# facebookresearch/SlowFast

Measured on AMD Instinct MI355X. Metric: clips/sec (fwd+bwd), SlowFast-8x8-R50 32x224^2 synthetic clips, per-GPU batch 32, higher is better.
Workload: dtype fp16; 1 GPU; SLOWFAST_8x8_R50: forward + cross_entropy loss + backward + sgd step, inputs resident in HBM, per-GPU batch 32; global_batch=32, parallelism=dp1, launch=hip-graph(fwd+bwd) + eager all-reduce/optimizer, optimizer=FlatOptimizer (fused unscale+norm+clip+update, dynamic loss scale on device)

## Files before the change

### include/sfamd.h

```cpp
#ifndef SFAMD_H
#define SFAMD_H
#include <stddef.h>
#include <stdint.h>
#ifdef __cplusplus
extern "C" {
#endif

#define SF_ABI_VERSION 34
typedef void* sf_stream_t;

typedef struct sf_conv_desc {
    int32_t N, Ci, Ti, Hi, Wi;
    int32_t Co, To, Ho, Wo;
    int32_t kT, kH, kW;
    int32_t sT, sH, sW;
    int32_t pT, pH, pW;
    int32_t dT, dH, dW;
    int32_t Cw;
    int32_t ldx, ldy;
    int32_t Cow;
} sf_conv_desc;

int sf_abi_version(void);
const char* sf_backend(void);
#define SF_ACT_FP16 0
#define SF_ACT_BF16_ID 1
int sf_act_dtype(void);
const char* sf_last_error(void);
const char* sf_build_id(void);

int sf_conv_weight_ld(const sf_conv_desc* d, int32_t* ldf, int32_t* ldd);
int sf_prep_weights(const sf_conv_desc* d, const float* w, void* wf, void* wd, sf_stream_t stream);
typedef struct sf_prep_item {
    const float* w;
    void* wf;
    void* wd;
    int32_t Co, Cow, Cw, Cp, taps, ldf, ldd;
    int32_t pad;
} sf_prep_item;
int sf_prep_item_fill(const sf_conv_desc* d, const float* w, void* wf, void* wd, sf_prep_item* item);
int64_t sf_prep_item_blocks(const sf_prep_item* item);
int sf_prep_weights_batch(const sf_prep_item* items, const int32_t* blk_item, const int32_t* blk_off, int32_t nblocks,
                          sf_stream_t stream);
int sf_conv_fwd_mtiles(const sf_conv_desc* d);
int sf_conv_fwd(const sf_conv_desc* d, const void* x, const void* wf, const float* in_scale, const float* in_shift,
                int in_relu, const float* bias, void* y, float* stat_part, sf_stream_t stream);
int sf_conv_fwd_fused(const sf_conv_desc* d, const void* x, const void* wf, const float* bias, const void* resid,
                      int32_t ldr, int out_relu, void* y, sf_stream_t stream);
int sf_conv_dgrad(const sf_conv_desc* d, const void* dy, const void* wd, const void* resid, int32_t ldr,
                  const void* resid_bits, void* dx, sf_stream_t stream);
int sf_conv_dgrad_bn(const sf_conv_desc* d, const void* dy, const void* wd, const void* resid, int32_t ldr,
                     const void* resid_bits, void* dx, const float* mask_scale, const float* mask_shift,
                     const void* mask_bits, const void* bn_y, int32_t bn_ldy, float* bn_part, int32_t bn_part_rows,
                     int32_t* bn_rows, sf_stream_t stream);
int64_t sf_conv_wgrad_workspace(const sf_conv_desc* d);
int64_t sf_conv_wgrad_rowtab_bytes(const sf_conv_desc* d);
int sf_conv_wgrad_rowtab(const sf_conv_desc* d, void* tab, sf_stream_t stream);
int sf_conv_wgrad(const sf_conv_desc* d, const void* x, const float* in_scale, const float* in_shift, int in_relu,
                  const void* dy, float* dw, float out_scale, int zero_first, void* workspace, int64_t workspace_bytes,
                  const void* rowtab, sf_stream_t stream);
int sf_conv_c_bwd_plan(const sf_conv_desc* d, int in_affine, int mask_bits, int32_t* tile_rows, int64_t* workspace_bytes);
int sf_conv_c_bwd(const sf_conv_desc* d, const void* dz, int32_t lddz, const void* mask_bits, const void* yc, int32_t ldyc,
                  const float* coef, const void* act, const void* wd, const float* bn_scale, const float* bn_shift,
                  const void* bn_y, int32_t bn_ldy, float* bn_part, int32_t bn_part_rows, int32_t* bn_rows, void* d_in,
                  int32_t ld_in, float* dw, float out_scale, int zero_first, void* workspace, int64_t workspace_bytes,
                  sf_stream_t stream);

int sf_bn_finalize(float* part, int32_t nblk, int32_t C, int32_t Creal, float count, const float* gamma, const float* beta,
                   float* running_mean, float* running_var, float momentum, float eps, float* scale, float* shift,
                   float* save_mean, float* save_rstd, sf_stream_t stream);
int sf_bn_act(int64_t M, int32_t C, const void* y, int32_t ldy, const float* scale, const float* shift, const void* r,
              int32_t ldr, const float* rscale, const float* rshift, int relu, void* out, int32_t ldo, void* mask_out,
              sf_stream_t stream);
int sf_bn_bwd_blocks(int64_t M, int32_t C);
int sf_bn_bwd_reduce(int64_t M, int32_t C, const void* dz, int32_t lddz, const void* zmask, int32_t ldm, const void* y,
                     int32_t ldy, const float* scale, const float* shift, int relu_self, float* part,
                     sf_stream_t stream);
int sf_bn_bwd_finalize(float* part, int32_t nblk, int32_t C, int32_t Creal, float count, const float* gamma, const float* mean,
                       const float* rstd, float inv_loss_scale, float* dgamma, float* dbeta, int accumulate,
                       float* coef, sf_stream_t stream);
int sf_bn_bwd_apply(int64_t M, int32_t C, const void* dz, int32_t lddz, const void* zmask, int32_t ldm, const void* y,
                    int32_t ldy, const float* scale, const float* shift, int relu_self, const float* coef, void* dy,
                    int32_t lddy, void* gout, int32_t ldg, sf_stream_t stream);

int sf_pool_fwd(int32_t N, int32_t T, int32_t H, int32_t W, int32_t C, int32_t kH, int32_t kW, int32_t sH, int32_t sW,
                int32_t pH, int32_t pW, const void* y, int32_t ldy, const float* scale, const float* shift, int relu,
                void* out, int32_t ldo, void* argmax, int32_t cls, sf_stream_t stream);
int sf_pool_bwd(int32_t N, int32_t T, int32_t H, int32_t W, int32_t C, int32_t kH, int32_t kW, int32_t sH, int32_t sW,
                int32_t pH, int32_t pW, const void* pooled, int32_t ldp, const void* argmax, int relu,
                const void* dout, int32_t lddo, void* g, int32_t ldg, int32_t cls, sf_stream_t stream);

int sf_pool3d_fwd(int32_t N, int32_t T, int32_t H, int32_t W, int32_t C, int32_t kT, int32_t kH, int32_t kW, const void* x,
                  int32_t ldx, void* out, int32_t ldo, void* argmax, sf_stream_t stream);
int sf_pool3d_bwd(int32_t N, int32_t T, int32_t H, int32_t W, int32_t C, int32_t kT, int32_t kH, int32_t kW,
                  const void* argmax, const void* dout, int32_t lddo, void* dx, int32_t lddx, sf_stream_t stream);

int sf_ncthw_to_cl(const float* x, int32_t N, int32_t C, int64_t S, int32_t Cp, void* out, sf_stream_t stream);
int sf_cl_to_ncthw(const void* x, int32_t ld, int32_t N, int32_t C, int64_t S, float* out, sf_stream_t stream);


int sf_bgemm(int64_t M, int32_t N, int32_t K, const void* A, int32_t lda, const void* W, int32_t ldw, const float* bias,
             const void* resid, int32_t ldr, void* Y, int32_t ldy, int32_t nbatch, int32_t bh, int64_t sa_b, int64_t sa_h,
             int64_t sw_b, int64_t sw_h, int64_t sy_b, int64_t sy_h, int64_t sr_b, int64_t sr_h, int32_t resid_row0,
             float alpha, sf_stream_t stream);
typedef struct sf_rows32 {
    const float* in;
    float* out;
    int32_t ld, period;
} sf_rows32;
int sf_gemm_rows32(int64_t M, int32_t N, int32_t K, const void* A, int32_t lda, const void* W, int32_t ldw, const float* bias,
                   const void* resid, int32_t ldr, void* Y, int32_t ldy, const sf_rows32* side, sf_stream_t stream);
int sf_bgemm_tn(int64_t M, int32_t R, int32_t Kc, const void* P, int32_t ldp, const void* X, int32_t ldx, void* Out,
                int32_t ldo, float scale, int32_t nbatch, int32_t bh, int64_t sp_b, int64_t sp_h, int64_t sx_b,
                int64_t sx_h, int64_t so_b, int64_t so_h, sf_stream_t stream);

int sf_layernorm_fwd(int64_t M, int32_t C, const void* x, int32_t ldx, const float* gamma, const float* beta, float eps,
                     void* y, int32_t ldy, float* mean, float* rstd, sf_stream_t stream);
int sf_layernorm_fwd_rows32(int64_t M, int32_t C, const void* x, int32_t ldx, const float* gamma, const float* beta, float eps,
                            void* y, int32_t ldy, float* mean, float* rstd, const sf_rows32* side, sf_stream_t stream);
int sf_layernorm_bwd_blocks(int64_t M, int32_t C);
int sf_layernorm_bwd(int64_t M, int32_t C, const void* dy, int32_t lddy, const void* x, int32_t ldx, const float* gamma,
                     const float* mean, const float* rstd, const void* resid, int32_t ldr, void* dx, int32_t lddx,
                     float* part, sf_stream_t stream);
int sf_layernorm_bwd_sums(int64_t M, int32_t C, const void* dy, int32_t lddy, const void* x, int32_t ldx, const float* gamma,
                          const float* mean, const float* rstd, const void* resid, int32_t ldr, void* dx, int32_t lddx,
                          float* part, sf_stream_t stream);
int sf_colsum_blocks(int64_t M, int32_t C);
int sf_colsum(int64_t M, int32_t C, const void* x, int32_t ldx, float* part, sf_stream_t stream);
int sf_colsum_finalize(float* part, int32_t nblk, int32_t C, int32_t fold, float* out0, float* out1, float scale,
                       int accumulate, sf_stream_t stream);
typedef struct sf_colfin_item {
    float* part;
    int32_t nblk, C, fold;
    float* out0;
    float* out1;
    float scale;
    int32_t accumulate;
    int32_t row_stride;
} sf_colfin_item;
int sf_colsum_finalize_batch(const sf_colfin_item* items, int32_t n, sf_stream_t stream);
int sf_rows_sum(const float* part, int32_t nblk, int64_t row_len, int64_t offset, int32_t n, float* out, float scale,
                int accumulate, sf_stream_t stream);
int sf_gelu_fwd(int64_t n, const void* h, void* a, sf_stream_t stream);
int sf_gelu_bwd(int64_t n, const void* h, const void* da, void* dh, sf_stream_t stream);

typedef struct sf_dw_desc {
    int32_t N, C, Cw, cls;
    int32_t Ti, Hi, Wi, To, Ho, Wo;
    int32_t kT, kH, kW, sT, sH, sW, pT, pH, pW;
// ... 196 lines not shown
```

### slowfast_amd/csrc/sf_api.hip

```cpp
#include "../../include/sfamd.h"
#include "sf_bn.h"
#include "sf_common.h"
#include "sf_igemm.h"
#include "sf_igemm2.h"
#include "sf_wgrad2.h"
#include "sf_cbwd.h"
#include "sf_pool.h"
#include "sf_dwconv.h"
#include "sf_dwsweep.h"
#include "sf_dwtemporal.h"
#include "sf_tokens.h"
#include "sf_x3d.h"
#include "sf_stem.h"
#include "sf_attn.h"
#include "sf_roi.h"
#include "sf_optim.h"
#include "sf_mixup.h"
#include "sf_erase.h"
#include "sf_pack.h"
#include "sf_sample.h"
#include "sf_color.h"
#include "sf_randaug.h"
#include "sf_sslcolor.h"
#include "sf_hog.h"
// ... 541 lines not shown
        }
    }
    IgemmParams p = gemm_params(gather_fwd(d, x, nullptr, nullptr, 0), d->N * d->To * d->Ho * d->Wo, wf, ldf, d->Co,
                                y, d->ldy, bias, resid, ldr);
    p.act_mode = out_relu ? 3 : 0;
    return run_igemm(p, is_pointwise(d), (hipStream_t)stream);
}

struct BnFuse {
    const float* scale; const float* shift; const void* bits;
    const void* y0; int32_t ld0; float* part0;
};
static int conv_dgrad_impl(const sf_conv_desc* d, const void* dy, const void* wd, const void* resid, int32_t ldr,
                           const void* resid_bits, void* dx, const BnFuse* bn, int32_t* bn_rows, sf_stream_t stream) {
    if (check_desc(d)) return -1;
    REQUIRE(dy && wd && dx, "sf_conv_dgrad: null pointer");
    REQUIRE(!resid || (ldr >= d->Ci && ldr % 8 == 0), "sf_conv_dgrad: bad residual pitch");
    int32_t ldf, ldd;
    sf_conv_weight_ld(d, &ldf, &ldd);
    IgemmParams p = gemm_params(gather_dgrad(d, dy), d->N * d->Ti * d->Hi * d->Wi, wd, ldd, d->Ci, dx, d->ldx, nullptr, resid, ldr);
    REQUIRE(!resid_bits || resid, "sf_conv_dgrad: resid_bits without a residual");
    p.resid_bits = (const uint8_t*)resid_bits;
    const bool fuse = bn && d->sT == 1 && d->sH == 1 && d->sW == 1;
    if (!resid && d->Co == 8 && d->To == d->Ti && d->Ho == d->Hi && d->Wo == d->Wi) {
        sf_conv_desc dd = *d;
        dd.Ci = d->Co; dd.Cw = d->Co; dd.Co = d->Ci; dd.Cow = 0;
        dd.pT = d->kT - 1 - d->pT; dd.pH = d->kH - 1 - d->pH; dd.pW = d->kW - 1 - d->pW;
        dd.ldx = d->ldy; dd.ldy = d->ldx;
        const StemPlan sp = plan_stem_fwd(&dd, true, fuse, cdiv(p.M, 128), fuse);
        if (sp.ok) {
            StemParams q = stem_fwd_params(&dd, sp, dy, wd, ldd, dx);
            const int S = d->kT * d->kH;
            q.wo0 = ((S - 1) * 3 + 2) * 8; q.wos = -24; q.wog = -8; q.kwc = 3;
            if (fuse) {
                q.bnb_y = (const f16*)bn->y0; q.bnb_ld = bn->ld0; q.bnb_scale = bn->scale; q.bnb_shift = bn->shift;
                q.bnb_bits = (const uint8_t*)bn->bits;
                q.stat_part = bn->part0; q.stat_rows = 0;
            }
            launch_stem_fwd(sp, q, (hipStream_t)stream);
            if (bn_rows) *bn_rows = fuse ? sp.ntiles : 0;
            return check_launch("stem_dgrad");
        }
    }
    if (fuse) {
        p.bnb_y = (const f16*)bn->y0; p.bnb_ld = bn->ld0; p.bnb_part = bn->part0;
        p.bnb_scale = bn->scale; p.bnb_shift = bn->shift; p.bnb_bits = (const uint8_t*)bn->bits;
    }
    GemmPlan g;
    const int rc = run_igemm(p, is_pointwise(d), (hipStream_t)stream, &g);
    if (bn_rows) *bn_rows = (fuse && g.bm > 0) ? cdiv(p.M, g.bm) : 0;
    return rc;
}

extern "C" int sf_conv_dgrad(const sf_conv_desc* d, const void* dy, const void* wd, const void* resid, int32_t ldr,
                             const void* resid_bits, void* dx, sf_stream_t stream) {
    return conv_dgrad_impl(d, dy, wd, resid, ldr, resid_bits, dx, nullptr, nullptr, stream);
}

extern "C" int sf_conv_dgrad_bn(const sf_conv_desc* d, const void* dy, const void* wd, const void* resid, int32_t ldr,
                                const void* resid_bits, void* dx, const float* mask_scale, const float* mask_shift,
                                const void* mask_bits, const void* bn_y, int32_t bn_ldy, float* bn_part, int32_t bn_part_rows,
                                int32_t* bn_rows, sf_stream_t stream) {
    REQUIRE(d && bn_y && bn_part && bn_rows, "sf_conv_dgrad_bn: null pointer");
    REQUIRE(mask_bits || (mask_scale && mask_shift), "sf_conv_dgrad_bn: a mask source is needed (mask_bits, or mask_scale + mask_shift)");
    REQUIRE(bn_ldy >= d->Ci && bn_ldy % 8 == 0 && ((uintptr_t)bn_y & 15) == 0, "sf_conv_dgrad_bn: bad bn_y pitch / alignment");
    REQUIRE((int64_t)bn_part_rows * 128 >= (int64_t)d->N * d->Ti * d->Hi * d->Wi,
            "sf_conv_dgrad_bn: the partial table needs ceil(positions / 128) rows of [2][Ci] floats");
    const BnFuse bn = {mask_scale, mask_shift, mask_bits, bn_y, bn_ldy, bn_part};
    return conv_dgrad_impl(d, dy, wd, resid, ldr, resid_bits, dx, &bn, bn_rows, stream);
}

static inline int wgrad1_bmw(int rows) { return rows >= 128 ? 128 : rows >= 64 ? 64 : rows >= 32 ? 32 : 16; }
static inline int wgrad1_ks(int bmw) { return bmw <= 32 ? 4 : 1; }
static void launch_wgrad1(int bmw, WgradParams& p, dim3 grid3, hipStream_t s) {
    p.tiles_k = grid3.x; p.tiles_c = grid3.y;
    const dim3 grid(grid3.x * grid3.y * grid3.z), block(SF_THREADS);
    switch (bmw) {
        case 128: hipLaunchKernelGGL((sf_wgrad_kernel<128, 64, 64, 1>), grid, block, 0, s, p); break;
        case 64: hipLaunchKernelGGL((sf_wgrad_kernel<64, 32, 64, 1>), grid, block, 0, s, p); break;
        case 32: hipLaunchKernelGGL((sf_wgrad_kernel<32, 32, 32, 4>), grid, block, 0, s, p); break;
        default: hipLaunchKernelGGL((sf_wgrad_kernel<16, 16, 32, 4>), grid, block, 0, s, p); break;
    }
}
static void launch_wgrad_reduce(const sf_conv_desc* d, const float* ws, int slabs, int Co_pad, int Kpad, bool slice4, float* dw,
                                float out_scale, int zero_first, hipStream_t s) {
    WgradReduceParams r;
    memset(&r, 0, sizeof(r));
    r.ws = ws; r.splits = slabs; r.Co = d->Cow ? d->Cow : d->Co; r.Co_pad = Co_pad; r.Kpad = Kpad;
    r.taps = d->kT * d->kH * d->kW; r.Ktot = r.taps * d->Ci; r.fdC = make_fastdiv(d->Ci); r.dw = dw; r.Cw = d->Cw;
    if (slice4) { r.slice4 = 1; r.Ktot = d->kT * d->kH * 32; }
    r.out_scale = out_scale; r.accumulate = zero_first ? 0 : 1;
    const int64_t total = (int64_t)r.Co * r.Kpad / 4;
    r.lanes = 1;
    while (r.lanes < 32 && r.lanes * 4 <= r.splits) r.lanes *= 2;
    hipLaunchKernelGGL(sf_wgrad_reduce_kernel, dim3(cdiv(total, SF_THREADS / r.lanes)), dim3(SF_THREADS), 0, s, r);
}

enum WgradPath { WGRAD_GEN1, WGRAD_ROWTAB, WGRAD_STEM };
struct WgradPlan {
    WgradPath path;
    bool thin, dual;
    int BMW, BKW, KS, tiles_k, tiles_c, Co_pad, Kpad;
    int nchunks, chunks_per_split;
    int rows_per_split, splits;
    int slabs;
    size_t tab_bytes, ws_bytes;
    StemPlan stem;
};
static WgradPlan plan_wgrad1(const sf_conv_desc* d) {
    WgradPlan w;
    memset(&w, 0, sizeof(w));
    w.path = WGRAD_GEN1;
    const int taps = d->kT * d->kH * d->kW;
    const int Ktot = taps * d->Ci;
    const int64_t M = (int64_t)d->N * d->To * d->Ho * d->Wo;
    w.BMW = wgrad1_bmw(d->Co); w.KS = wgrad1_ks(w.BMW);
    w.tiles_k = cdiv(Ktot, 128);
    w.tiles_c = cdiv(d->Co, w.BMW);
    w.Kpad = w.tiles_k * 128;
    w.Co_pad = w.tiles_c * w.BMW;
    w.nchunks = cdiv(M, 32);
    const int64_t slab = (int64_t)w.Co_pad * w.Kpad * 4;
    static const int target = tune_knob("SF_WGRAD_BLOCKS", 1024);
    int splits = cdiv(target, (int64_t)w.tiles_k * w.tiles_c);
    const int64_t cap = (256ll << 20) / slab;
    if (splits > cap) splits = (int)(cap < 1 ? 1 : cap);
    const int nstages = cdiv(w.nchunks, w.KS);
    if (splits > nstages) splits = nstages;
    if (splits < 1) splits = 1;
    w.chunks_per_split = cdiv(nstages, splits) * w.KS;
    w.splits = cdiv(w.nchunks, w.chunks_per_split);
    w.slabs = w.splits;
    w.ws_bytes = (size_t)slab * w.splits;
    return w;
}

static bool plan_wgrad2(const sf_conv_desc* d, WgradPlan& w) {
    if (test_hook("SF_WGRAD2", 1) == 0) return false;
    const int mink = test_hook("SF_WGRAD2_MINK", 192);
    const int minrows = test_hook("SF_WGRAD2_MINROWS", 4096);
    const int taps = d->kT * d->kH * d->kW;
    const int target = test_hook("SF_WGRAD2_BLOCKS", 512);
    const int Ktot = taps * d->Ci;
    const int64_t M = (int64_t)d->N * d->To * d->Ho * d->Wo;
    if (taps > SF_I2_MAXTAPS || M < minrows) return false;
    if ((d->kT - 1) * d->dT > 127 || (d->kH - 1) * d->dH > 127 || (d->kW - 1) * d->dW > 127) return false;
    if (d->Co <= 32) {
        if (test_hook("SF_WGRAD2T", 1) == 0) return false;
        const int minrows_t = test_hook("SF_WGRAD2T_MINROWS", 16384);
        if (M < minrows_t) return false;
        w.thin = true;
        w.BMW = d->Co <= 16 ? 16 : 32;
        w.BKW = Ktot <= 32 ? 32 : 128;
        w.tiles_k = cdiv(Ktot, w.BKW);
        w.tiles_c = 1;
        w.Kpad = w.tiles_k * w.BKW;
        w.Co_pad = w.BMW;
        const int target_t = test_hook("SF_WGRAD2T_BLOCKS", w.BKW == 128 ? 512 : w.BMW == 32 ? 768 : 1024);
        int splits = target_t / w.tiles_k;
        if (splits < 1) splits = 1;
        w.rows_per_split = roundup(cdiv(M, splits), 128);
        w.splits = cdiv(M, w.rows_per_split);
        w.tab_bytes = ((size_t)M * 8 + 255) / 256 * 256 + 1280;
        w.ws_bytes = w.tab_bytes + (size_t)w.Co_pad * w.Kpad * 4 * w.splits;
        w.slabs = w.splits;
        w.path = WGRAD_ROWTAB;
        return true;
    }
    if (Ktot < mink) return false;
    w.BMW = d->Co > 64 ? 128 : 64;
    w.tiles_k = cdiv(Ktot, 256);
    w.tiles_c = cdiv(d->Co, w.BMW);
    w.Kpad = w.tiles_k * 256;
    w.Co_pad = w.tiles_c * w.BMW;
    int splits = target / (w.tiles_k * w.tiles_c);
    const int64_t slab = (int64_t)w.Co_pad * w.Kpad * 4;
    const int64_t cap = (256ll << 20) / slab;
    if (splits > cap) splits = (int)(cap < 1 ? 1 : cap);
    if (splits < 1) splits = 1;
    w.dual = false;
    if (splits >= 2 && test_hook("SF_WGRAD2_DUAL", 1) != 0) {
        const int tiles = w.tiles_k * w.tiles_c;
        const int pairs = (target / 2) / tiles;
        const int64_t steps = cdiv(cdiv(M, splits), 32);
        if (pairs >= 1 && 2 * pairs * 10 >= (2 * pairs < splits ? splits : 2 * pairs) * 9 && steps <= test_hook("SF_WGRAD2_DUAL_STEPS", 80)) {
            w.dual = true;
            if (2 * pairs < splits) splits = 2 * pairs;
        }
    }
    w.rows_per_split = roundup(cdiv(M, splits), 32);
    w.splits = cdiv(M, w.rows_per_split);
    if (w.splits < 2) w.dual = false;
    w.slabs = w.dual ? cdiv(w.splits, 2) : w.splits;
    w.tab_bytes = ((size_t)M * 8 + 255) / 256 * 256 + 1280;
    w.ws_bytes = w.tab_bytes + (size_t)slab * w.splits;
    w.path = WGRAD_ROWTAB;
    return true;
}
static WgradPlan plan_conv_wgrad(const sf_conv_desc* d, bool in_affine) {
    const StemPlan sp = plan_stem(d);
    WgradPlan w;
    memset(&w, 0, sizeof(w));
    if (in_affine || !(sp.ok || plan_wgrad2(d, w))) w = plan_wgrad1(d);
    else if (sp.ok) {
        w.path = WGRAD_STEM;
        w.slabs = sp.wg_blocks * sp.wgroups; w.Co_pad = 16; w.Kpad = sp.Kpad; w.ws_bytes = sp.ws_bytes;
    }
    w.stem = sp;
    return w;
}

static void launch_rowtab(const sf_conv_desc* d, void* tab, hipStream_t s) {
    RowtabParams t;
    memset(&t, 0, sizeof(t));
    t.tab = (i32x2*)tab;
    t.M = d->N * d->To * d->Ho * d->Wo;
    t.fdW = make_fastdiv(d->Wo); t.fdH = make_fastdiv(d->Ho); t.fdT = make_fastdiv(d->To);
    t.sT = d->Ti; t.sH = d->Hi; t.sW = d->Wi;
    t.strT = d->sT; t.strH = d->sH; t.strW = d->sW; t.padT = d->pT; t.padH = d->pH; t.padW = d->pW;
    t.ntaps = d->kT * d->kH * d->kW;
    int ti = 0;
    for (int kt = 0; kt < d->kT; ++kt)
        for (int kh = 0; kh < d->kH; ++kh)
            for (int kw = 0; kw < d->kW; ++kw, ++ti) {
                t.dt[ti] = (int8_t)(kt * d->dT); t.dh[ti] = (int8_t)(kh * d->dH); t.dw[ti] = (int8_t)(kw * d->dW);
            }
    hipLaunchKernelGGL(sf_wgrad2_rowtab_kernel, dim3(cdiv(t.M, SF_THREADS)), dim3(SF_THREADS), 0, s, t);
}

extern "C" int64_t sf_conv_wgrad_rowtab_bytes(const sf_conv_desc* d) {
    if (check_desc(d)) return -1;
    return (int64_t)plan_conv_wgrad(d, false).tab_bytes;
}

extern "C" int sf_conv_wgrad_rowtab(const sf_conv_desc* d, void* tab, sf_stream_t stream) {
    if (check_desc(d)) return -1;
    REQUIRE(tab && (uintptr_t)tab % 16 == 0, "sf_conv_wgrad_rowtab: tab must be a 16-byte aligned device pointer");
    REQUIRE(plan_conv_wgrad(d, false).path == WGRAD_ROWTAB, "sf_conv_wgrad_rowtab: this geometry does not take the row-table kernel (sf_conv_wgrad_rowtab_bytes == 0)");
    launch_rowtab(d, tab, (hipStream_t)stream);
    return check_launch("wgrad_rowtab");
}

extern "C" int64_t sf_conv_wgrad_workspace(const sf_conv_desc* d) {
    if (check_desc(d)) return -1;
    const int64_t plain = (int64_t)plan_conv_wgrad(d, false).ws_bytes, affine = (int64_t)plan_conv_wgrad(d, true).ws_bytes;
    return plain > affine ? plain : affine;
}

extern "C" int sf_conv_wgrad(const sf_conv_desc* d, const void* x, const float* in_scale, const float* in_shift,
                             int in_relu, const void* dy, float* dw, float out_scale, int zero_first,
                             void* workspace, int64_t workspace_bytes, const void* rowtab, sf_stream_t stream) {
    if (check_desc(d)) return -1;
    REQUIRE(x && dy && dw && workspace, "sf_conv_wgrad: null pointer");
    REQUIRE((in_scale == nullptr) == (in_shift == nullptr), "sf_conv_wgrad: in_scale/in_shift must come together");
    REQUIRE(!in_scale || d->Ci <= 512, "sf_conv_wgrad: fused input BatchNorm supports Ci <= 512 (got %d)", d->Ci);
    hipStream_t s = (hipStream_t)stream;
    GatherSide gk = gather_fwd(d, x, in_scale, in_shift, in_relu);
    const WgradPlan w = plan_conv_wgrad(d, in_scale != nullptr);
    REQUIRE(workspace_bytes >= (int64_t)w.ws_bytes, "sf_conv_wgrad: workspace too small (%lld < %lld bytes)",
            (long long)workspace_bytes, (long long)w.ws_bytes);
    float* slabs = (float*)((char*)workspace + w.tab_bytes);
    if (w.path == WGRAD_ROWTAB) {
        REQUIRE(((uintptr_t)x | (uintptr_t)dy | (uintptr_t)workspace) % 16 == 0, "sf_conv_wgrad: operands must be 16-byte aligned");
        Wgrad2Params q;
        memset(&q, 0, sizeof(q));
        int ti = 0;
        for (int kt = 0; kt < d->kT; ++kt)
            for (int kh = 0; kh < d->kH; ++kh)
                for (int kw = 0; kw < d->kW; ++kw, ++ti) q.dlin[ti] = (kt * d->dT * d->Hi + kh * d->dH) * d->Wi + kw * d->dW;
        if (!rowtab) launch_rowtab(d, workspace, s);
        else REQUIRE((uintptr_t)rowtab % 16 == 0, "sf_conv_wgrad: rowtab must be 16-byte aligned");
        q.x = (const f16*)x; q.ldx = d->ldx; q.C = d->Ci;
        q.dy = (const f16*)dy; q.ldy = d->ldy; q.Co = d->Co;
        q.M = d->N * d->To * d->Ho * d->Wo; q.Ktot = gk.Ktot;
        q.rowtab = (const i32x2*)(rowtab ? rowtab : workspace);
        q.ws = slabs; q.Co_pad = w.Co_pad; q.Kpad = w.Kpad;
        q.tiles_k = w.tiles_k; q.tiles_c = w.tiles_c; q.rows_per_split = w.rows_per_split;
        q.stage_stride = (w.thin && tune_knob("SF_WGRAD2T_RR", 1) != 0) ? w.splits : 0;
        const dim3 grid((unsigned)(w.tiles_k * w.tiles_c * w.slabs));
        if (sf_trace()) fprintf(stderr, "[sfamd] wgrad2: M=%d Co=%d K=%d tiles %dx%d splits %d%s\n", q.M, q.Co, q.Ktot, w.tiles_c, w.tiles_k, w.splits,
                                w.dual ? " (two per workgroup)" : "");
        if (w.thin) {
            if (w.BMW == 16 && w.BKW == 128) hipLaunchKernelGGL((sf_wgrad2t_kernel<16, 128, 2>), grid, dim3(256), 0, s, q);
            else if (w.BMW == 32 && w.BKW == 128) hipLaunchKernelGGL((sf_wgrad2t_kernel<32, 128, 2>), grid, dim3(256), 0, s, q);
            else if (w.BMW == 16) hipLaunchKernelGGL((sf_wgrad2t_kernel<16, 32, 3>), grid, dim3(256), 0, s, q);
            else hipLaunchKernelGGL((sf_wgrad2t_kernel<32, 32, 3>), grid, dim3(256), 0, s, q);
        } else if (w.dual) {
            if (w.BMW == 128) hipLaunchKernelGGL((sf_wgrad2_kernel<128, true>), grid, dim3(1024), 0, s, q);
            else hipLaunchKernelGGL((sf_wgrad2_kernel<64, true>), grid, dim3(1024), 0, s, q);
        } else {
            if (w.BMW == 128) hipLaunchKernelGGL((sf_wgrad2_kernel<128>), grid, dim3(512), 0, s, q);
            else hipLaunchKernelGGL((sf_wgrad2_kernel<64>), grid, dim3(512), 0, s, q);
        }
    } else if (w.path == WGRAD_STEM) {
        const StemPlan& sp = w.stem;
        StemParams q = stem_params(d, sp, x);
        q.dy = (const f16*)dy; q.ws = (float*)workspace;
        if (sf_trace()) fprintf(stderr, "[sfamd] stem_wgrad: %d workgroups x %d tiles\n", sp.wg_blocks, sp.tiles_per_block);
        static const bool stem_plain = tune_knob("SF_STEM_XCD", 1) == 0;
        q.plain_order = stem_plain ? 1 : 0;
        const dim3 grid(sp.wg_blocks), block(SF_STEM_WG_THREADS);
        if (d->Co <= 8 && sp.small) hipLaunchKernelGGL((sf_stem_wgrad_kernel<8, SF_STEM_CHUNKS_SMALL>), grid, block, 0, s, q);
        else if (d->Co <= 8) hipLaunchKernelGGL((sf_stem_wgrad_kernel<8, SF_STEM_CHUNKS>), grid, block, 0, s, q);
        else if (sp.small) hipLaunchKernelGGL((sf_stem_wgrad_kernel<16, SF_STEM_CHUNKS_SMALL>), grid, block, 0, s, q);
        else hipLaunchKernelGGL((sf_stem_wgrad_kernel<16, SF_STEM_CHUNKS>), grid, block, 0, s, q);
    } else {
        REQUIRE(w.splits <= 65535, "sf_conv_wgrad: too many splits");
        WgradParams p;
        memset(&p, 0, sizeof(p));
        p.g = gk;
        p.dy = (const f16*)dy; p.ldy = d->ldy; p.Co = d->Co;
        p.M = d->N * d->To * d->Ho * d->Wo;
        p.ws = (float*)workspace; p.Co_pad = w.Co_pad; p.Kpad = w.Kpad;
        p.nchunks = w.nchunks; p.chunks_per_split = w.chunks_per_split;
        launch_wgrad1(w.BMW, p, dim3(w.tiles_k, w.tiles_c, w.splits), s);
    }
    if (check_launch("wgrad")) return -1;
    launch_wgrad_reduce(d, slabs, w.slabs, w.Co_pad, w.Kpad, w.path == WGRAD_STEM && w.stem.thin3, dw, out_scale, zero_first, s);
    return check_launch("wgrad_reduce");
}

struct CbwdPlan {
    bool ok;
    int cip, cop, R;
    size_t ws_bytes;
};
#define SF_CBWD_MAX_WGS 1024
template <int CIP, int COP>
static void cbwd_fill(CbwdPlan& w) {
    using K = CbwdCfg<CIP, COP>;
    w.R = K::R;
    w.ws_bytes = (size_t)SF_CBWD_MAX_WGS * COP * CIP * 4;
}
#define SF_CBWD_FOR_SHAPE(cip, cop, ...)                                                         \
    do {                                                                                         \
        if ((cip) == 16 && (cop) == 32) { constexpr int CIP_ = 16, COP_ = 32; __VA_ARGS__; }            \
        else if ((cip) == 16 && (cop) == 64) { constexpr int CIP_ = 16, COP_ = 64; __VA_ARGS__; }       \
        else if ((cip) == 16 && (cop) == 128) { constexpr int CIP_ = 16, COP_ = 128; __VA_ARGS__; }     \
        else if ((cip) == 16 && (cop) == 256) { constexpr int CIP_ = 16, COP_ = 256; __VA_ARGS__; }     \
        else if ((cip) == 32 && (cop) == 32) { constexpr int CIP_ = 32, COP_ = 32; __VA_ARGS__; }       \
        else if ((cip) == 32 && (cop) == 64) { constexpr int CIP_ = 32, COP_ = 64; __VA_ARGS__; }       \
        else if ((cip) == 32 && (cop) == 128) { constexpr int CIP_ = 32, COP_ = 128; __VA_ARGS__; }     \
        else if ((cip) == 32 && (cop) == 256) { constexpr int CIP_ = 32, COP_ = 256; __VA_ARGS__; }     \
        else if ((cip) == 64 && (cop) == 32) { constexpr int CIP_ = 64, COP_ = 32; __VA_ARGS__; }       \
        else if ((cip) == 64 && (cop) == 64) { constexpr int CIP_ = 64, COP_ = 64; __VA_ARGS__; }       \
        else if ((cip) == 64 && (cop) == 128) { constexpr int CIP_ = 64, COP_ = 128; __VA_ARGS__; }     \
        else { constexpr int CIP_ = 64, COP_ = 256; __VA_ARGS__; }                                      \
    } while (0)
static CbwdPlan plan_cbwd(const sf_conv_desc* d, bool in_affine, bool mask_bits) {
    CbwdPlan w;
    memset(&w, 0, sizeof(w));
    if (test_hook("SF_CBWD", 1) == 0) return w;
    if (d->kT != 1 || d->kH != 1 || d->kW != 1 || d->sT != 1 || d->sH != 1 || d->sW != 1 || d->pT || d->pH || d->pW) return w;
    if (d->To != d->Ti || d->Ho != d->Hi || d->Wo != d->Wi) return w;
    if (d->Ci % 8 || d->Ci > 64 || d->Co % 32 || d->Co > 256) return w;
    if (in_affine || !mask_bits) return w;
    w.cip = d->Ci <= 16 ? 16 : d->Ci <= 32 ? 32 : 64;
    w.cop = d->Co <= 32 ? 32 : d->Co <= 64 ? 64 : d->Co <= 128 ? 128 : 256;
    SF_CBWD_FOR_SHAPE(w.cip, w.cop, (cbwd_fill<CIP_, COP_>(w)));
    w.ok = true;
    return w;
}

extern "C" int sf_conv_c_bwd_plan(const sf_conv_desc* d, int in_affine, int mask_bits, int32_t* tile_rows,
                                  int64_t* workspace_bytes) {
    if (check_desc(d)) return -1;
    const CbwdPlan w = plan_cbwd(d, in_affine != 0, mask_bits != 0);
    if (tile_rows) *tile_rows = w.ok ? 128 : 0;
    if (workspace_bytes) *workspace_bytes = w.ok ? (int64_t)w.ws_bytes : 0;
    return w.ok ? 1 : 0;
}

extern "C" int sf_conv_c_bwd(const sf_conv_desc* d, const void* dz, int32_t lddz, const void* mask_bits, const void* yc,
                             int32_t ldyc, const float* coef, const void* act, const void* wd, const float* bn_scale,
                             const float* bn_shift, const void* bn_y, int32_t bn_ldy, float* bn_part, int32_t bn_part_rows,
                             int32_t* bn_rows, void* d_in, int32_t ld_in, float* dw, float out_scale, int zero_first,
                             void* workspace, int64_t workspace_bytes, sf_stream_t stream) {
    if (check_desc(d)) return -1;
    REQUIRE(dz && mask_bits && yc && coef && act && wd && d_in && dw && workspace, "sf_conv_c_bwd: null pointer");
    const CbwdPlan w = plan_cbwd(d, false, true);
    REQUIRE(w.ok, "sf_conv_c_bwd: this geometry keeps sf_bn_bwd_apply + sf_conv_wgrad + sf_conv_dgrad_bn (sf_conv_c_bwd_plan == 0)");
    REQUIRE(lddz >= d->Co && lddz % 8 == 0 && ldyc >= d->Co && ldyc % 8 == 0 && ld_in >= d->Ci && ld_in % 8 == 0,
            "sf_conv_c_bwd: bad row pitch");
    REQUIRE((((uintptr_t)dz | (uintptr_t)yc | (uintptr_t)act | (uintptr_t)wd | (uintptr_t)d_in | (uintptr_t)workspace) & 15) == 0,
            "sf_conv_c_bwd: operands must be 16-byte aligned");
    REQUIRE(workspace_bytes >= (int64_t)w.ws_bytes, "sf_conv_c_bwd: workspace too small (%lld < %lld bytes)",
            (long long)workspace_bytes, (long long)w.ws_bytes);
    const int64_t M = (int64_t)d->N * d->Ti * d->Hi * d->Wi;
    const int ntiles = cdiv(M, 128);
    const bool fuse = bn_part != nullptr;
    if (fuse) {
        REQUIRE(bn_scale && bn_shift && bn_y && bn_rows, "sf_conv_c_bwd: the fused reduction needs bn_scale, bn_shift, bn_y and bn_rows");
        REQUIRE(bn_ldy >= d->Ci && bn_ldy % 8 == 0 && ((uintptr_t)bn_y & 15) == 0, "sf_conv_c_bwd: bad bn_y pitch / alignment");
        REQUIRE(bn_part_rows >= ntiles, "sf_conv_c_bwd: the partial table needs ceil(positions / tile_rows) rows of [2][Ci] floats");
    }
    int32_t ldf, ldd;
    sf_conv_weight_ld(d, &ldf, &ldd);
    CbwdParams p;
    memset(&p, 0, sizeof(p));
    p.M = (int)M; p.Ci = d->Ci; p.Co = d->Co;
    p.dz = (const f16*)dz; p.lddz = lddz; p.bits = (const uint8_t*)mask_bits; p.yc = (const f16*)yc; p.ldyc = ldyc;
    p.coef = coef; p.act = (const f16*)act; p.ldact = d->ldx; p.wd = (const f16*)wd; p.ldw = ldd;
    if (fuse) { p.bnb_y = (const f16*)bn_y; p.bnb_ld = bn_ldy; p.bnb_scale = bn_scale; p.bnb_shift = bn_shift; p.bnb_part = bn_part; }
    p.dx = (f16*)d_in; p.lddx = ld_in; p.ws = (float*)workspace; p.tiles128 = ntiles;
    int wgs;
    const WgradPlan w2 = plan_conv_wgrad(d, false);
    const int forced = test_hook("SF_CBWD_WGS", 0);
    if (forced > 0) {
        wgs = forced < SF_CBWD_MAX_WGS ? forced : SF_CBWD_MAX_WGS;
        p.rps = roundup(cdiv(M, wgs), 32);
        wgs = cdiv(M, p.rps);
    } else if (w2.path == WGRAD_ROWTAB && w2.thin && w2.splits <= SF_CBWD_MAX_WGS) {
        wgs = w2.splits; p.rps = 0;
    } else {
        const WgradPlan w1 = plan_wgrad1(d);
        wgs = w1.splits; p.rps = w1.chunks_per_split * 32;
        REQUIRE(wgs <= SF_CBWD_MAX_WGS, "sf_conv_c_bwd: %d splits", wgs);
    }
    hipStream_t s = (hipStream_t)stream;
    SF_CBWD_FOR_SHAPE(w.cip, w.cop, hipLaunchKernelGGL((sf_cbwd_kernel<CIP_, COP_>), dim3(wgs), dim3(SF_THREADS), 0, s, p));
    if (check_launch("conv_c_bwd")) return -1;
    if (bn_rows) *bn_rows = fuse ? ntiles : 0;
    launch_wgrad_reduce(d, (const float*)workspace, wgs, w.cop, w.cip, false, dw, out_scale, zero_first, s);
    return check_launch("conv_c_bwd_reduce");
}

static RowTile make_rowtile(int64_t M, int C, int max_blocks, dim3& grid) {
    RowTile rt;
    rt.M = (int)M; rt.C = C;
    const int G = C / 8;
    const int TG = G < SF_THREADS ? G : SF_THREADS;
    const int rpi = SF_THREADS / TG;
    int passes = cdiv(M, (int64_t)rpi * max_blocks);
    if (passes < 1) passes = 1;
    rt.rows_per_block = rpi * passes;
    grid = dim3(cdiv(M, rt.rows_per_block), cdiv(G, SF_THREADS));
    return rt;
}
static int check_rows(const char* who, int64_t M, int C) {
    REQUIRE(M > 0 && M < (1ll << 31), "%s: bad row count", who);
    REQUIRE(C > 0 && C % 8 == 0, "%s: C must be a positive multiple of 8 (got %d)", who, C);
    return 0;
}

static const int kFoldAbove = tune_knob("SF_FOLD_ABOVE", 2048);
static int fold_partials(float* part, int& nblk, int C, hipStream_t s) {
    if (nblk <= kFoldAbove || nblk <= 256) return 1;
    const int group = nblk <= 2048 ? 16 : nblk <= 8192 ? 32 : 64;
    const int cols = 2 * C;
    dim3 grid(cdiv(cols, SF_THREADS), cdiv(nblk, group));
    hipLaunchKernelGGL(sf_part_fold_kernel, grid, dim3(SF_THREADS), 0, s, part, nblk, cols, group);
    nblk = cdiv(nblk, group);
    return group;
}

extern "C" int sf_bn_finalize(float* part, int32_t nblk, int32_t C, int32_t Creal, float count, const float* gamma,
                              const float* beta, float* running_mean, float* running_var, float momentum, float eps,
                              float* scale, float* shift, float* save_mean, float* save_rstd, sf_stream_t stream) {
    REQUIRE(gamma && beta && scale && shift, "sf_bn_finalize: null pointer");
    REQUIRE(nblk > 0 ? part != nullptr : (running_mean && running_var), "sf_bn_finalize: missing statistics source");
    REQUIRE(Creal > 0 && Creal <= C, "sf_bn_finalize: Creal must be in (0, C]");
    BnFinalizeParams p;
    p.row_stride = nblk > 0 ? fold_partials(part, nblk, C, (hipStream_t)stream) : 1;
    p.part = part; p.nblk = nblk; p.C = C; p.Creal = Creal; p.count = count; p.gamma = gamma; p.beta = beta;
    p.running_mean = running_mean; p.running_var = running_var; p.momentum = momentum; p.eps = eps;
    p.scale = scale; p.shift = shift; p.save_mean = save_mean; p.save_rstd = save_rstd;
    hipLaunchKernelGGL(sf_bn_finalize_kernel, dim3(cdiv(C, SF_FIN_CH)), dim3(sf_fin_threads(p.nblk)), 0, (hipStream_t)stream, p);
    return check_launch("bn_finalize");
}

extern "C" int sf_bn_act(int64_t M, int32_t C, const void* y, int32_t ldy, const float* scale, const float* shift,
                         const void* r, int32_t ldr, const float* rscale, const float* rshift, int relu, void* out,
                         int32_t ldo, void* mask_out, sf_stream_t stream) {
    if (check_rows("sf_bn_act", M, C)) return -1;
    REQUIRE(y && out, "sf_bn_act: null pointer");
    BnActParams p;
    dim3 grid;
    p.rt = make_rowtile(M, C, 8192, grid);
    p.y = (const f16*)y; p.ldy = ldy; p.scale = scale; p.shift = shift;
    p.r = (const f16*)r; p.ldr = ldr; p.rscale = rscale; p.rshift = rshift;
    p.relu = relu; p.out = (f16*)out; p.ldo = ldo; p.mask_out = (uint8_t*)mask_out;
    hipLaunchKernelGGL(sf_bn_act_kernel, grid, dim3(SF_THREADS), 0, (hipStream_t)stream, p);
    return check_launch("bn_act");
}

static const int kBwdBlocks = tune_knob("SF_BN_BWD_BLOCKS", 1024);
extern "C" int sf_bn_bwd_blocks(int64_t M, int32_t C) {
    if (check_rows("sf_bn_bwd_blocks", M, C)) return -1;
    dim3 grid;
    make_rowtile(M, C, kBwdBlocks, grid);
    return (int)grid.x;
}

extern "C" int sf_bn_bwd_reduce(int64_t M, int32_t C, const void* dz, int32_t lddz, const void* zmask, int32_t ldm,
                                const void* y, int32_t ldy, const float* scale, const float* shift, int relu_self,
                                float* part, sf_stream_t stream) {
    if (check_rows("sf_bn_bwd_reduce", M, C)) return -1;
    REQUIRE(dz && y && part, "sf_bn_bwd_reduce: null pointer");
    REQUIRE(!relu_self || (scale && shift), "sf_bn_bwd_reduce: relu_self needs scale/shift");
    BnBwdReduceParams p;
    dim3 grid;
    p.rt = make_rowtile(M, C, kBwdBlocks, grid);
    p.dz = (const f16*)dz; p.lddz = lddz; p.zmask = (const f16*)zmask; p.ldm = ldm;
    p.y = (const f16*)y; p.ldy = ldy; p.scale = scale; p.shift = shift; p.relu_self = relu_self; p.part = part;
    hipLaunchKernelGGL(sf_bn_bwd_reduce_kernel, grid, dim3(SF_THREADS), 0, (hipStream_t)stream, p);
    return check_launch("bn_bwd_reduce");
}
// ... 2379 lines not shown
```

### slowfast_amd/csrc/sf_igemm.h

```cpp
#pragma once
#include "sf_common.h"

struct IgemmParams {
    GatherSide g;
    int M;
    const f16* wmat;
    int ldw;
    int Nout;
    int ksteps;
    f16* y;
    int ldy;
    const float* bias;
    const f16* resid;
    int ldr;
    float* stat_part;
    int ntiles_n;
    int bh;
    int64_t sa_b, sa_h, sw_b, sw_h, sy_b, sy_h, sr_b, sr_h;
    int act_mode;
    f16* act_aux;
    int ld_aux;
    int resid_row0;
    const uint8_t* resid_bits;
    float alpha;
// ... 320 lines not shown
            ok[u] = idx < BM * CG && m < p.M && ecol < p.Nout;
            rok[u] = ok[u] && resid && m >= p.resid_row0;
            if constexpr (F32R) {
                uint32_t srow;
                if (f32_row(p.f32, m, srow)) rok[u] = false;
            }
            L[u].rbits = 0xffu; L[u].bbits = 0u;
            if (rok[u]) {
                L[u].r = ld16(resid + (int64_t)m * p.ldr + ecol);
                if (p.resid_bits) L[u].rbits = p.resid_bits[(int64_t)m * (p.Nout >> 3) + (ecol >> 3)];
            }
            if (ok[u] && bnb && p.bnb_y) {
                L[u].y = ld16(p.bnb_y + (int64_t)m * p.bnb_ld + ecol);
                if (p.bnb_bits) L[u].bbits = p.bnb_bits[(int64_t)m * (p.Nout >> 3) + (ecol >> 3)];
            }
        }
#pragma unroll
        for (int u = 0; u < CH; ++u) {
            if (!ok[u]) continue;
            const int idx = tid + (it0 + u) * SF_THREADS;
            const int row = idx / CG, m = m0 + row;
            f16x8 v = ld16(stg + row * STG_LD + ecg * 8);
            if (rok[u]) {
#pragma unroll
                for (int e = 0; e < 8; ++e) {
                    const f16 r = ((L[u].rbits >> e) & 1u) ? L[u].r[e] : (f16)0.f;
                    v[e] = (f16)((float)v[e] + (float)r);
                }
            }
            if (p.act_mode == 2) {
                const f16x8 h = ld16(p.act_aux + (int64_t)m * p.ld_aux + ecol);
#pragma unroll
                for (int e = 0; e < 8; ++e) v[e] = (f16)((float)v[e] * gelu_df((float)h[e]));
            }
            if (p.act_mode == 3) {
#pragma unroll
                for (int e = 0; e < 8; ++e) v[e] = v[e] > (f16)0.f ? v[e] : (f16)0.f;
            }
            st16(yout + (int64_t)m * p.ldy + ecol, v);
            if (p.act_mode == 1) {
                f16x8 a;
#pragma unroll
                for (int e = 0; e < 8; ++e) a[e] = (f16)gelu_f((float)v[e]);
                st16(p.act_aux + (int64_t)m * p.ld_aux + ecol, a);
            }
            if (bnb && p.bnb_y) bnb_accumulate(v, L[u].y, bsc, bsh, bsg, bsgy, p.bnb_bits != nullptr, L[u].bbits);
            else if (bnb) {
#pragma unroll
                for (int e = 0; e < 8; ++e) bsg[e] += (float)v[e];
            }
        }
    }
    if (bnb) bnb_reduce_store<4, CG>(bsg, bsgy, reinterpret_cast<float*>(smem), p.bnb_part + (int64_t)mt * 2 * p.Nout, n0, p.Nout);
}

struct WgradParams {
    GatherSide g;
    const f16* dy;
    int ldy;
    int Co;
    int M;
    float* ws;
    int Co_pad, Kpad;
    int nchunks;
    int chunks_per_split;
    int tiles_k, tiles_c;
    int bh;
    int64_t sp_b, sp_h, sx_b, sx_h, so_b, so_h;
    f16* out16; int ldo; float out_scale;
};

struct WgradReduceParams {
    const float* ws;
    int splits, Co, Co_pad, Kpad, Ktot;
    FastDiv fdC;
    float* dw;
    int Cw, taps;
    float out_scale;
    int accumulate;
    int lanes;
    int slice4;
};

__global__ __launch_bounds__(SF_THREADS) void sf_wgrad_reduce_kernel(WgradReduceParams p) {
    __shared__ f32x4 s_acc[SF_THREADS];
    const int L = p.lanes, E = SF_THREADS / L;
    const int e = threadIdx.x % E, z0 = threadIdx.x / E;
    const int64_t total = (int64_t)p.Co * p.Kpad;
    const int64_t slab = (int64_t)p.Co_pad * p.Kpad;
    const int64_t idx = ((int64_t)blockIdx.x * E + e) * 4;
    f32x4 a0 = {0.f, 0.f, 0.f, 0.f}, a1 = a0, a2 = a0, a3 = a0;
    if (idx < total) {
        const float* src = p.ws + idx;
        int z = z0;
        for (; z + 3 * L < p.splits; z += 4 * L) {
            const f32x4 v0 = *reinterpret_cast<const f32x4*>(src + (int64_t)z * slab);
            const f32x4 v1 = *reinterpret_cast<const f32x4*>(src + (int64_t)(z + L) * slab);
            const f32x4 v2 = *reinterpret_cast<const f32x4*>(src + (int64_t)(z + 2 * L) * slab);
            const f32x4 v3 = *reinterpret_cast<const f32x4*>(src + (int64_t)(z + 3 * L) * slab);
            a0 += v0; a1 += v1; a2 += v2; a3 += v3;
        }
        for (; z < p.splits; z += L) a0 += *reinterpret_cast<const f32x4*>(src + (int64_t)z * slab);
    }
    s_acc[threadIdx.x] = (a0 + a1) + (a2 + a3);
    __syncthreads();
    for (int half = L >> 1; half >= 1; half >>= 1) {
        if (z0 < half) s_acc[threadIdx.x] += s_acc[threadIdx.x + half * E];
        __syncthreads();
    }
    if (z0 == 0 && idx < total) {
        const int co = (int)(idx / p.Kpad), kcol0 = (int)(idx % p.Kpad);
        const f32x4 r = s_acc[threadIdx.x];
#pragma unroll
        for (int j = 0; j < 4; ++j) {
            const int kcol = kcol0 + j;
            if (kcol < p.Ktot) {
                uint32_t tap, ci;
                fd_divmod((uint32_t)kcol, p.fdC, tap, ci);
                if (p.slice4) {
                    if ((tap & 3u) == 3u) continue;
                    tap = (tap >> 2) * 3u + (tap & 3u);
                }
                if (ci < (uint32_t)p.Cw) {
                    float* dst = p.dw + ((int64_t)co * p.Cw + ci) * p.taps + tap;
                    const float v = r[j] * p.out_scale;
                    *dst = p.accumulate ? *dst + v : v;
                }
            }
        }
    }
}

template <class V>
__device__ __forceinline__ f16x4 as_f16x4(V v) {
    f16x4 o;
    __builtin_memcpy(&o, &v, 8);
    return o;
}

struct TapPos {
    int dt, dh, dw;
    uint32_t c0;
    bool valid;
};
__device__ __forceinline__ TapPos decode_tap(const GatherSide& g, uint32_t k0) {
    TapPos t;
    t.valid = k0 < (uint32_t)g.Ktot;
    uint32_t tap, kt, kh, kw, q;
    fd_divmod(t.valid ? k0 : 0u, g.fdC, tap, t.c0);
    fd_divmod(tap, g.fdkW, q, kw);
    fd_divmod(q, g.fdkH, kt, kh);
    t.dt = (int)kt * g.dilT; t.dh = (int)kh * g.dilH; t.dw = (int)kw * g.dilW;
    return t;
}
__device__ __forceinline__ bool gather_offset_tap(const GatherSide& g, const RowPos& r, const TapPos& tp, int64_t& off) {
    if (!r.valid || !tp.valid) return false;
    const int t = r.bt + tp.dt, h = r.bh + tp.dh, w = r.bw + tp.dw;
    if ((unsigned)t >= (unsigned)g.sT || (unsigned)h >= (unsigned)g.sH || (unsigned)w >= (unsigned)g.sW) return false;
    off = ((((int64_t)r.n * g.sT + t) * g.sH + h) * g.sW + w) * (int64_t)g.ld + tp.c0;
    return true;
}

template <int BMW, int WM, int WN, int KS>
__global__ __launch_bounds__(SF_THREADS) void sf_wgrad_kernel(WgradParams p) {
    constexpr int BNW = 128, BKM = 32, ROWS = BKM * KS;
    constexpr int WAVES_N = BNW / WN, WAVES_M = BMW / WM;
    static_assert(WAVES_M * WAVES_N == 4, "4 waves per workgroup");
    constexpr int TM = WM / 16, TN = WN / 16;
    constexpr int LDA = BMW + 16, LDB = BNW + 16;
    constexpr int BUF = ROWS * (LDA + LDB);
    constexpr int NBUF = KS == 1 ? 2 : 1;
    constexpr int NA = (ROWS * (BMW / 8) + SF_THREADS - 1) / SF_THREADS;
    constexpr int NX = 2 * KS;

    __shared__ __attribute__((aligned(16))) f16 smem[NBUF * BUF];
    __shared__ __attribute__((aligned(16))) float s_scale[512];
    __shared__ __attribute__((aligned(16))) float s_shift[512];

    const int tid = threadIdx.x;
    const int lane = tid & 63, wave = tid >> 6;
    const int wm = wave / WAVES_N, wn = wave % WAVES_N;
    const uint32_t wg = xcd_remap(blockIdx.x, gridDim.x);
    const int bx = (int)(wg % (uint32_t)p.tiles_k);
    const int by = (int)((wg / (uint32_t)p.tiles_k) % (uint32_t)p.tiles_c);
    const int bz = (int)(wg / ((uint32_t)p.tiles_k * (uint32_t)p.tiles_c));
    const int n0 = bx * BNW, c0 = by * BMW;
    const GatherSide& g = p.g;
    const bool has_tf = g.scale != nullptr;
    if (has_tf) {
        for (int c = tid; c < g.C; c += SF_THREADS) {
            s_scale[c] = g.scale[c];
            s_shift[c] = g.shift[c];
        }
    }
    const f16* x_src = g.src;
    const f16* dy_src = p.dy;
    f16* out16 = p.out16;
    const int nstages = (p.nchunks + KS - 1) / KS;
    int sb = bz * (p.chunks_per_split / KS);
    int se = sb + p.chunks_per_split / KS;
    if (p.bh > 0) {
        const int zb = bz / p.bh, zj = bz % p.bh;
        dy_src += zb * p.sp_b + zj * p.sp_h;
        x_src += zb * p.sx_b + zj * p.sx_h;
        out16 += zb * p.so_b + zj * p.so_h;
        sb = 0;
        se = nstages;
    }
    if (se > nstages) se = nstages;

    f16x8 ra[NA], rb[NX];
    bool rb_ok[NX];
    const TapPos tp = decode_tap(g, (uint32_t)(n0 + (tid & 15) * 8));

// ... 125 lines not shown
```

### slowfast_amd/engine.py

```python
import functools
import os

import torch

from . import lib as _sflib

from . import ops

_f16 = _sflib.act_dtype()
_listeners = []
FORCE_WEIGHT_PREP = False
PARAM_EPOCH = 0
PACK_RECORD = None
PACK_PLAN = os.environ.get("SF_PACK_PLAN", "1") != "0"
BN_FUSE_REDUCE = os.environ.get("SF_BN_FUSE_REDUCE", "1") != "0"
CAT_IN_PLACE = os.environ.get("SF_CAT_IN_PLACE", "1") != "0"
SEGMENTS = None


class _Segments:
    def __init__(self):
        self.cuts = []

    def cut(self, tensors):
# ... 547 lines not shown
        N, Cs, T, H, W = x_s.shape
        Cf = yf.shape[1]
        assert tuple(yf.shape) == (N, Cf, T, H, W), "lateral connection does not match the Slow pathway shape"
        cat = getattr(x_s, "_sf_cat", None)
        if cat is not None and tuple(cat.shape) == (N, Cs + Cf, T, H, W) and cat.data_ptr() == x_s.data_ptr():
            pass
        else:
            cat = ops.cl_empty((N, Cs + Cf, T, H, W), x_s.device)
            ops.bn_act(x_s, out=cat[:, :Cs])
        ops.bn_act(yf, st.scale, st.shift, relu=True, out=cat[:, Cs:])
        if CAPTURE is not None:
            CAPTURE.append({"kind": "fuse", "mod": mod, "raw": [yf], "bn": [(st.scale, st.shift)]})
        ctx.mod, ctx.yf, ctx.st, ctx.Cs = mod, yf, st, Cs
        ctx.save_for_backward(x_f)
        return cat, x_f.view_as(x_f)

    @staticmethod
    @delivers_grads
    def backward(ctx, dcat, dxf):
        unit = ctx.mod._unit
        (x_f,) = ctx.saved_tensors
        dcat = as_cl(dcat)
        dyf = unit.bn_backward(dcat[:, ctx.Cs:], ctx.yf, ctx.st, relu_self=True)
        need_dx = ctx.needs_input_grad[1]
        dx_f = unit.backward(x_f, None, dyf, need_dx=need_dx, resid=as_cl(dxf) if dxf is not None else None)
        _notify(unit.params())
        ctx.yf = None
        dx_s = dcat[:, :ctx.Cs] if ctx.needs_input_grad[0] else None
        return (dx_s, dx_f, None) + param_grads(ctx, 3)


class ResBlockFn(torch.autograd.Function):

    @staticmethod
    def forward(ctx, x, mod, *params):
        record_params(ctx, params)
        ctx.prev_bn = getattr(x, "_sf_block_bn", None) if BN_FUSE_REDUCE else None
        x = as_cl(x)
        units, P = mod.branch2._chain, mod._proj
        tr = mod.training
        raw, bn, act, h = [], [], [], x
        for i, u in enumerate(units):
            h, st = u.forward(h, None, tr)
            raw.append(h)
            bn.append(st)
            if i + 1 < len(units):
                h = ops.bn_act(h, st.scale, st.shift, relu=True)
                act.append(h)
        yc, sc = raw[-1], bn[-1]
        out_view, cat = None, None
        extra = getattr(mod, "_cat_extra", 0)
        if extra and CAT_IN_PLACE:
            N_, C_, T_, H_, W_ = yc.shape
            cat = ops.cl_empty((N_, C_ + extra, T_, H_, W_), x.device)
            out_view = cat[:, :C_]
        if P is not None:
            y1, s1 = P.forward(x, None, tr)
            out, bits = ops.bn_act(yc, sc.scale, sc.shift, relu=True, resid=y1, rscale=s1.scale, rshift=s1.shift,
                                   want_mask=True, out=out_view)
        else:
            y1, s1 = None, None
            out, bits = ops.bn_act(yc, sc.scale, sc.shift, relu=True, resid=x, want_mask=True, out=out_view)
        if cat is not None:
            out._sf_cat = cat
        if CAPTURE is not None:
            CAPTURE.append({"kind": "resblock", "mod": mod, "raw": list(raw), "bn": [(b.scale, b.shift) for b in bn], "out": out})
        ctx.mod = mod
        ctx.raw = (raw, y1, act, bits)
        ctx.bn = (bn, s1)
        ctx.save_for_backward(x)
        if BN_FUSE_REDUCE and tr:
            out._sf_block_bn = {"bits": bits, "y0": yc, "sync": _sync_of(units[-1].bn) is not None}
        return out

    @staticmethod
    @delivers_grads
    def backward(ctx, dout):
        mod = ctx.mod
        units, P = mod.branch2._chain, mod._proj
        (x,) = ctx.saved_tensors
        raw, y1, act, bits = ctx.raw
        bn, s1 = ctx.bn
        last = len(units) - 1
        part_c = tagged_bn_part(dout, raw[last])
        dout = as_cl(dout)
        need_dx = ctx.needs_input_grad[0]
        cgeom = units[last].fused_c_geom(act[last - 1]) if last > 0 else None
        if cgeom is None:
            dy = units[last].bn_backward(dout, raw[last], bn[last], zmask=bits, part=part_c)
        if P is not None:
            dy1 = P.bn_backward(dout, y1, s1, zmask=bits)
        for i in range(last, 0, -1):
            part = None
            if i == last and cgeom is not None:
                inner = (raw[i - 1], bn[i - 1]) if BN_FUSE_REDUCE and _sync_of(units[i - 1].bn) is None else None
                d_in, part = units[i].fused_c_backward(cgeom, act[i - 1], dout, raw[i], bn[i], bits, part=part_c, bn_fuse=inner)
            elif BN_FUSE_REDUCE and _sync_of(units[i - 1].bn) is None:
                d_in, part = units[i].backward(act[i - 1], None, dy, need_dx=True, bn_fuse=(raw[i - 1], bn[i - 1]))
            else:
                d_in = units[i].backward(act[i - 1], None, dy, need_dx=True)
            dy = units[i - 1].bn_backward(d_in, raw[i - 1], bn[i - 1], relu_self=True, part=part)
        prev = ctx.prev_bn if need_dx else None
        if prev is not None and prev["sync"]:
            prev = None
        if P is not None:
            dx1 = P.backward(x, None, dy1, need_dx=need_dx)
            dx = units[0].backward(x, None, dy, need_dx=need_dx, resid=dx1, bn_fuse=prev)
        else:
            dx = units[0].backward(x, None, dy, need_dx=need_dx, resid=dout, resid_bits=bits, bn_fuse=prev)
        if prev is not None:
            dx, pc = dx
            if pc is not None:
                tag_bn_part(dx, prev["y0"], pc)
        _notify(mod._param_list)
        ctx.raw = ctx.bn = ctx.prev_bn = None
        return (dx, None) + param_grads(ctx, 2)


CUT_BACKWARD = False
_cut_bn_tags = {}


def retag_cut_grad(g):
    tag = _cut_bn_tags.pop(g.data_ptr(), None)
    if tag is not None and getattr(g, "_sf_bn_part", None) is None and tag[2] == g.data_ptr() and tag[3] == g._version:
        g._sf_bn_part = tag


def tag_bn_part(dx, y0, part):
    dx._sf_bn_part = (y0.data_ptr(), part, dx.data_ptr(), dx._version)
    if CUT_BACKWARD:
        _cut_bn_tags[dx.data_ptr()] = dx._sf_bn_part


def tagged_bn_part(dout, y0):
    tag = getattr(dout, "_sf_bn_part", None)
    if tag is None or tag[0] != y0.data_ptr() or tag[2] != dout.data_ptr() or tag[3] != dout._version:
        return None
    return tag[1]


class ConvBNActFn(torch.autograd.Function):

    @staticmethod
    def forward(ctx, x, unit, relu, training, *params):
        record_params(ctx, params)
        x = as_cl(x)
        y, st = unit.forward(x, None, training)
        out = ops.bn_act(y, st.scale, st.shift, relu=relu)
        if CAPTURE is not None:
            CAPTURE.append({"kind": "convbnact", "mod": None, "raw": [y], "bn": [(st.scale, st.shift)], "out": out})
        ctx.unit, ctx.relu, ctx.y, ctx.st = unit, relu, y, st
        ctx.save_for_backward(x)
        return out

    @staticmethod
    @delivers_grads
    def backward(ctx, dout):
        unit = ctx.unit
        (x,) = ctx.saved_tensors
        dy = unit.bn_backward(as_cl(dout), ctx.y, ctx.st, relu_self=ctx.relu)
        dx = unit.backward(x, None, dy, need_dx=ctx.needs_input_grad[0])
        _notify(unit.params())
        ctx.y = None
        return (dx, None, None, None) + param_grads(ctx, 4)
```

### slowfast_amd/lib.py

```python
import ctypes
import os
from ctypes import POINTER, Structure, c_char_p, c_float, c_int, c_int32, c_int64, c_void_p

_HERE = os.path.dirname(os.path.abspath(__file__))
ABI_VERSION = 34
ACT_MODE = os.environ.get("SF_ACT_DTYPE", "fp16").lower()
if ACT_MODE not in ("fp16", "bf16"):
    raise ValueError(f"SF_ACT_DTYPE={ACT_MODE!r}: expected fp16 or bf16")
DEFAULT_LIBRARY = os.path.join(_HERE, "libsfamd.so" if ACT_MODE == "fp16" else "libsfamd_bf16.so")


def act_dtype():
    import torch
    return torch.float16 if ACT_MODE == "fp16" else torch.bfloat16


def act_eps():
    return 2.0 ** -11 if ACT_MODE == "fp16" else 2.0 ** -8


class ConvDesc(Structure):

    _fields_ = [(n, c_int32) for n in (
        "N", "Ci", "Ti", "Hi", "Wi", "Co", "To", "Ho", "Wo", "kT", "kH", "kW", "sT", "sH", "sW",
        "pT", "pH", "pW", "dT", "dH", "dW", "Cw", "ldx", "ldy", "Cow")]


class PrepItem(Structure):

    _fields_ = [("w", c_void_p), ("wf", c_void_p), ("wd", c_void_p)] + [(n, c_int32) for n in (
        "Co", "Cow", "Cw", "Cp", "taps", "ldf", "ldd", "pad")]


class DwDesc(Structure):

    _fields_ = [(n, c_int32) for n in (
        "N", "C", "Cw", "cls", "Ti", "Hi", "Wi", "To", "Ho", "Wo", "kT", "kH", "kW", "sT", "sH", "sW",
        "pT", "pH", "pW", "ldx", "ldy", "Cwreal")]


class Rows32(Structure):

    _fields_ = [("in_", c_void_p), ("out", c_void_p), ("ld", c_int32), ("period", c_int32)]


class ColFinItem(Structure):

    _fields_ = [("part", c_void_p), ("nblk", c_int32), ("C", c_int32), ("fold", c_int32), ("out0", c_void_p),
                ("out1", c_void_p), ("scale", c_float), ("accumulate", c_int32), ("row_stride", c_int32)]


class AttnDesc(Structure):

    _fields_ = [(n, c_int32) for n in (
        "B", "heads", "D", "cls", "Nq", "qT", "qH", "qW", "Nk", "kT", "kH", "kW", "rows_h", "rows_w", "rows_t")]


_P = c_void_p
_F = c_void_p
_SIGNATURES = {
    "sf_abi_version": (c_int, []),
    "sf_backend": (c_char_p, []),
    "sf_act_dtype": (c_int, []),
    "sf_last_error": (c_char_p, []),
    "sf_build_id": (c_char_p, []),
    "sf_conv_weight_ld": (c_int, [POINTER(ConvDesc), POINTER(c_int32), POINTER(c_int32)]),
    "sf_prep_weights": (c_int, [POINTER(ConvDesc), _F, _P, _P, _P]),
    "sf_prep_item_fill": (c_int, [POINTER(ConvDesc), _F, _P, _P, POINTER(PrepItem)]),
    "sf_prep_item_blocks": (c_int64, [POINTER(PrepItem)]),
    "sf_prep_weights_batch": (c_int, [_P, _P, _P, c_int32, _P]),
    "sf_conv_fwd_mtiles": (c_int, [POINTER(ConvDesc)]),
    "sf_conv_fwd": (c_int, [POINTER(ConvDesc), _P, _P, _F, _F, c_int, _F, _P, _F, _P]),
    "sf_conv_fwd_fused": (c_int, [POINTER(ConvDesc), _P, _P, _F, _P, c_int32, c_int, _P, _P]),
    "sf_conv_dgrad": (c_int, [POINTER(ConvDesc), _P, _P, _P, c_int32, _P, _P, _P]),
    "sf_conv_dgrad_bn": (c_int, [POINTER(ConvDesc), _P, _P, _P, c_int32, _P, _P, _P, _P, _P, _P, c_int32, _P, c_int32,
                                 POINTER(c_int32), _P]),
    "sf_conv_wgrad_workspace": (c_int64, [POINTER(ConvDesc)]),
    "sf_conv_wgrad_rowtab_bytes": (c_int64, [POINTER(ConvDesc)]),
    "sf_conv_wgrad_rowtab": (c_int, [POINTER(ConvDesc), _P, _P]),
    "sf_conv_wgrad": (c_int, [POINTER(ConvDesc), _P, _F, _F, c_int, _P, _F, c_float, c_int, _P, c_int64, _P, _P]),
    "sf_conv_c_bwd_plan": (c_int, [POINTER(ConvDesc), c_int, c_int, POINTER(c_int32), POINTER(c_int64)]),
    "sf_conv_c_bwd": (c_int, [POINTER(ConvDesc), _P, c_int32, _P, _P, c_int32, _F, _P, _P, _F, _F, _P, c_int32, _F, c_int32,
                              POINTER(c_int32), _P, c_int32, _F, c_float, c_int, _P, c_int64, _P]),
    "sf_bn_finalize": (c_int, [_F, c_int32, c_int32, c_int32, c_float, _F, _F, _F, _F, c_float, c_float, _F, _F, _F, _F, _P]),
    "sf_bn_act": (c_int, [c_int64, c_int32, _P, c_int32, _F, _F, _P, c_int32, _F, _F, c_int, _P, c_int32, _P, _P]),
    "sf_bn_bwd_blocks": (c_int, [c_int64, c_int32]),
    "sf_flat_blocks": (c_int, [c_int64]),
    "sf_flat_sumsq": (c_int, [_F, c_int64, _F, _P]),
    "sf_step_control": (c_int, [_F, c_int32, _F, c_float, c_float, c_int, c_float, c_float, c_int32, _P]),
    "sf_flat_sgd": (c_int, [_F, _F, _F, _P, _P, _P, c_int32, _F, _P, _P, c_int32, c_float, c_float, c_float, c_int, _P]),
    "sf_flat_adamw": (c_int, [_F, _F, _F, _F, _P, _P, _P, c_int32, _F, _P, _P, c_int32, c_float, c_float, c_float, c_float, _P]),
    "sf_flat_sgd_tab": (c_int, [_F, _F, _F, _P, _P, _P, c_int32, _F, _F, _F, c_float, c_float, c_float, c_int, _P]),
    "sf_flat_adamw_tab": (c_int, [_F, _F, _F, _F, _P, _P, _P, c_int32, _F, _F, _F, c_float, c_float, c_float, c_float, _P]),
    "sf_flat_lars_trust": (c_int, [_F, _F, _P, _P, _P, c_int32, _P, c_int32, _F, _F, _P, _F, c_float, c_float, c_float, _P]),
    "sf_bn_bwd_reduce": (c_int, [c_int64, c_int32, _P, c_int32, _P, c_int32, _P, c_int32, _F, _F, c_int, _F, _P]),
    "sf_bn_bwd_finalize": (c_int, [_F, c_int32, c_int32, c_int32, c_float, _F, _F, _F, c_float, _F, _F, c_int, _F, _P]),
    "sf_bn_bwd_apply": (c_int, [c_int64, c_int32, _P, c_int32, _P, c_int32, _P, c_int32, _F, _F, c_int, _F, _P,
                                c_int32, _P, c_int32, _P]),
    "sf_pool_fwd": (c_int, [c_int32] * 11 + [_P, c_int32, _F, _F, c_int, _P, c_int32, _P, c_int32, _P]),
    "sf_pool_bwd": (c_int, [c_int32] * 11 + [_P, c_int32, _P, c_int, _P, c_int32, _P, c_int32, c_int32, _P]),
    "sf_pool3d_fwd": (c_int, [c_int32] * 8 + [_P, c_int32, _P, c_int32, _P, _P]),
    "sf_pool3d_bwd": (c_int, [c_int32] * 8 + [_P, _P, c_int32, _P, c_int32, _P]),
    "sf_ncthw_to_cl": (c_int, [_F, c_int32, c_int32, c_int64, c_int32, _P, _P]),
    "sf_cl_to_ncthw": (c_int, [_P, c_int32, c_int32, c_int32, c_int64, _F, _P]),
    "sf_bgemm": (c_int, [c_int64, c_int32, c_int32, _P, c_int32, _P, c_int32, _F, _P, c_int32, _P, c_int32, c_int32,
                         c_int32] + [c_int64] * 8 + [c_int32, c_float, _P]),
    "sf_bgemm_tn": (c_int, [c_int64, c_int32, c_int32, _P, c_int32, _P, c_int32, _P, c_int32, c_float, c_int32, c_int32]
                    + [c_int64] * 6 + [_P]),
    "sf_layernorm_fwd": (c_int, [c_int64, c_int32, _P, c_int32, _F, _F, c_float, _P, c_int32, _F, _F, _P]),
    "sf_gemm_rows32": (c_int, [c_int64, c_int32, c_int32, _P, c_int32, _P, c_int32, _F, _P, c_int32, _P, c_int32,
                               POINTER(Rows32), _P]),
    "sf_layernorm_fwd_rows32": (c_int, [c_int64, c_int32, _P, c_int32, _F, _F, c_float, _P, c_int32, _F, _F,
                                        POINTER(Rows32), _P]),
    "sf_layernorm_bwd_blocks": (c_int, [c_int64, c_int32]),
    "sf_layernorm_bwd": (c_int, [c_int64, c_int32, _P, c_int32, _P, c_int32, _F, _F, _F, _P, c_int32, _P, c_int32, _F, _P]),
    "sf_layernorm_bwd_sums": (c_int, [c_int64, c_int32, _P, c_int32, _P, c_int32, _F, _F, _F, _P, c_int32, _P, c_int32, _F, _P]),
    "sf_colsum_blocks": (c_int, [c_int64, c_int32]),
    "sf_colsum": (c_int, [c_int64, c_int32, _P, c_int32, _F, _P]),
    "sf_colsum_finalize": (c_int, [_F, c_int32, c_int32, c_int32, _F, _F, c_float, c_int, _P]),
    "sf_colsum_finalize_batch": (c_int, [POINTER(ColFinItem), c_int32, _P]),
    "sf_rows_sum": (c_int, [_F, c_int32, c_int64, c_int64, c_int32, _F, c_float, c_int, _P]),
    "sf_gelu_fwd": (c_int, [c_int64, _P, _P, _P]),
    "sf_gelu_bwd": (c_int, [c_int64, _P, _P, _P, _P]),
    "sf_dwconv_fwd_blocks": (c_int, [POINTER(DwDesc)]),
    "sf_dwconv_fwd_sample_rows": (c_int, [POINTER(DwDesc)]),
    "sf_dwconv_pair_ok": (c_int, [POINTER(DwDesc)]),
    "sf_dwconv_fwd_pair": (c_int, [POINTER(DwDesc), _P, _P, _F, _F, _P, _P, _P]),
    "sf_dwconv_dgrad_pair": (c_int, [POINTER(DwDesc), _P, _P, _F, _F, _P, _P, _P]),
    "sf_dwconv_wgrad_pair": (c_int, [POINTER(DwDesc), _P, _P, _P, _P, _F, _F, c_float, c_int, c_int, _P, c_int64, _P]),
    "sf_dwconv_fwd": (c_int, [POINTER(DwDesc), _P, _F, _P, _F, _P]),
    "sf_dwconv_dgrad": (c_int, [POINTER(DwDesc), _P, _F, _P, _P]),
    "sf_dwconv_dgrad_sum_rows": (c_int, [POINTER(DwDesc)]),
    "sf_dwconv_dgrad_sums": (c_int, [POINTER(DwDesc), _P, _F, _P, _F, _P]),
    "sf_dwconv_wgrad_workspace": (c_int64, [POINTER(DwDesc)]),
    "sf_dwconv_wgrad": (c_int, [POINTER(DwDesc), _P, _P, _F, c_float, c_int, _P, c_int64, _P]),
    "sf_relpos_gather": (c_int, [POINTER(AttnDesc), _P, c_int32, _P, _P, _P, _F, _P]),
    "sf_relpos_scatter": (c_int, [POINTER(AttnDesc), _F, _P, _P, _P, _P, c_int32, _P]),
    "sf_relpos_pack": (c_int, [_F, _F, _F, c_int32, c_int32, c_int32, c_int32, c_int32, _P, _P, _P]),
    "sf_relpos_unpack": (c_int, [_F, c_int32, c_int32, c_int32, c_int32, _F, _F, _F, c_int32, c_int32, c_int32, _P]),
    "sf_softmax_fwd": (c_int, [POINTER(AttnDesc), _P, c_int32, c_float, _F, _P]),
    "sf_softmax_bwd": (c_int, [POINTER(AttnDesc), _P, _P, c_int32, c_float, _F, _P]),
    "sf_attn_fwd": (c_int, [POINTER(AttnDesc), _P, c_int32, _P, _P, c_int32, c_float, _F, _P, c_int32, _P, c_int32, _F, _P]),
    "sf_attn_bwd_workspace": (c_int64, [POINTER(AttnDesc)]),
    "sf_attn_bwd": (c_int, [POINTER(AttnDesc), _P, c_int32, _P, _P, c_int32, c_float, _F, _P, c_int32, _P, _P, c_int32, _F,
                            _F, _P, c_int32, _P, _P, c_int32, _F, _P, c_int64, _P]),
    "sf_tmean_fwd": (c_int, [c_int32, c_int32, c_int64, c_int32, _P, c_int32, _F, _P]),
    "sf_tmean_bwd": (c_int, [c_int32, c_int32, c_int64, c_int32, _F, _P, c_int32, _P]),
    "sf_roi_align_max_fwd": (c_int, [c_int32, c_int32, c_int32, c_int32, c_int32, c_int32, c_float, c_int32, _F, _F, _F,
                                     c_int32, c_int32, _P, _P]),
    "sf_roi_align_max_bwd": (c_int, [c_int32, c_int32, c_int32, c_int32, c_int32, c_int32, c_float, c_int32, _F, _F,
                                     c_int32, c_int32, _P, _F, _P]),
    "sf_gemm_act": (c_int, [c_int64, c_int32, c_int32, _P, c_int32, _P, c_int32, _F, _P, c_int32, c_int32, _P, c_int32, _P]),
    "sf_gemm_act_colsum": (c_int, [c_int64, c_int32, c_int32, _P, c_int32, _P, c_int32, _F, _P, c_int32, c_int32, _P, c_int32, _P, c_int32, POINTER(c_int32), _P]),
    "sf_pack_clip_u8": (c_int, [_P, c_int32, c_int32, c_int32, c_int32, _P, c_int32, c_float, c_float, c_float, c_float,
                                c_float, c_float, c_int32, _P, _P]),
    "sf_mix_clip_f32": (c_int, [_F, _F, c_int32, c_int32, c_int32, c_int32, c_int32, c_int32, c_float, c_float, c_int32, c_int32,
                                c_int32, c_int32, _P]),
    "sf_pack_clip_u8_mix": (c_int, [_P, c_int32, c_int32, c_int32, c_int32, _P, c_int32, c_float, c_float, c_float, c_float,
                                    c_float, c_float, c_int32, _P, c_int32, c_float, c_float, c_int32, c_int32, c_int32, c_int32,
                                    _P]),
    "sf_mix_targets": (c_int, [_P, c_int32, c_int32, c_float, c_float, c_float, c_float, _F, _P]),
    "sf_erase_clip_f32": (c_int, [_F, _F, c_int32, c_int32, c_int32, c_int32, c_int32, c_int32, _P, _P, c_int32, c_int32, _P]),
    "sf_pack_clip_u8_aug": (c_int, [_P, c_int32, c_int32, c_int32, c_int32, _P, c_int32, c_float, c_float, c_float, c_float,
# ... 122 lines not shown
```

### slowfast_amd/mvit_engine.py

```python
import math
import os

import torch

from . import lib as _sflib

from . import engine, tokens
from . import engine as _engine
from .engine import _grad_dest, _notify, param_grads

_f16 = _sflib.act_dtype()

def _pair_kv(plan):
    return plan.gq is None


RESID32 = os.environ.get("SF_MVIT_RESID32", "1") != "0"
RESID32_FULL = os.environ.get("SF_MVIT_RESID32", "1") == "full"


class ResidSide:

    def __init__(self, cls32=None, full32=None):
        self.cls32, self.full32 = cls32, full32

    def reader(self, N):
        return (1, self.full32) if self.full32 is not None else (N, self.cls32)

    def cls_rows(self):
        return self.cls32 if self.full32 is None else self.full32[:, 0].contiguous()


def _sum_side(src, B, N, C, full, device):
    if full:
        dst = torch.empty((B, N, C), dtype=torch.float32, device=device)
        return (1, src.full32 if src is not None else None, dst), ResidSide(full32=dst)
    dst = torch.empty((B, C), dtype=torch.float32, device=device)
    return (N, src.cls_rows() if src is not None else None, dst), ResidSide(cls32=dst)


def _bias_from_parts(dy, db, accumulate, parts):
    if not parts or all(p is None for p in parts):
        tokens.bias_grad(dy, db, accumulate=accumulate)
        return
    C = dy.shape[-1] // len(parts)
    for i, part in enumerate(parts):
        dst = db[i * C:(i + 1) * C]
        if part is None:
            tokens.bias_grad(dy[..., i * C:(i + 1) * C], dst, accumulate=accumulate)
        else:
            tokens.colsum_finalize(part, C, C, dst, None, 1.0, accumulate)


class LinearUnit:

    def __init__(self, lin):
        self.lin = lin
        self._key, self._w, self._wt, self._planned = None, None, None, False

    def _ops(self, fresh=False):
        w = self.lin.weight
        key = (w.data_ptr(), w._version, w.device, _engine.PARAM_EPOCH)
        if (fresh and engine.FORCE_WEIGHT_PREP and not self._planned) or self._key != key:
            wd = w.detach()
            self._w = wd.to(_f16)
            self._wt = wd.t().contiguous().to(_f16)
            self._key = key
            N, K = w.shape
            if _engine.PACK_RECORD is not None and N % 32 == 0 and K % 32 == 0 and w.is_contiguous():
                _engine.PACK_RECORD.append((self, None, True))
        return self._w, self._wt

    def pack_item(self, geom, need_dgrad):
        from . import ops
        w = self.lin.weight
        N, K = w.shape
        g = ops.ConvGeom((1, K, 1, 1, 1), N, 1)
        assert g.ldf == K and g.ldd == N
        return (w, g.desc(K, N), torch.empty((N, K), dtype=_f16, device=w.device),
                torch.empty((K, N), dtype=_f16, device=w.device))

    def pack_assign(self, geom, wf, wd):
        w = self.lin.weight
        self._w, self._wt, self._planned = wf, wd, True
        self._key = (w.data_ptr(), w._version, w.device, _engine.PARAM_EPOCH)

    def forward(self, x, resid=None, out=None, side=None):
        w, _ = self._ops(fresh=True)
        return tokens.gemm(x, w, bias=self.lin.bias, resid=resid, out=out, side=side)

    def forward_gelu(self, x):
        w, _ = self._ops(fresh=True)
        return tokens.gemm_gelu(x, w, bias=self.lin.bias)

    def backward_through_gelu(self, x, dy, h, consumer_bias=None, bias_done=False):
        lin = self.lin
        if lin.weight.requires_grad:
            dw, zero_first = _grad_dest(lin.weight)
            tokens.linear_wgrad(x, dy, dw, zero_first=zero_first)
        if lin.bias is not None and lin.bias.requires_grad and not bias_done:
            db, zero_first = _grad_dest(lin.bias)
            tokens.bias_grad(dy, db, accumulate=not zero_first)
        _, wt = self._ops()
        if consumer_bias is not None and consumer_bias.requires_grad:
            dcb, zf = _grad_dest(consumer_bias)
            return tokens.gemm_gelu_grad(dy, wt, h, dbias=dcb, accumulate=not zf), True
        return tokens.gemm_gelu_grad(dy, wt, h), False

    def backward(self, x, dy, need_dx=True, resid=None, out=None, bias_done=False):
        lin = self.lin
        if lin.weight.requires_grad:
            dw, zero_first = _grad_dest(lin.weight)
            tokens.linear_wgrad(x, dy, dw, zero_first=zero_first)
        if lin.bias is not None and lin.bias.requires_grad and not bias_done:
            db, zero_first = _grad_dest(lin.bias)
            _bias_from_parts(dy, db, not zero_first, getattr(dy, "_sf_bias_parts", None))
        if not need_dx:
            return None
        _, wt = self._ops()
        return tokens.gemm(dy, wt, resid=resid, out=out)

    def bias_sum_dest(self):
        b = self.lin.bias
        if b is None or not b.requires_grad:
            return None
        dest, zero_first = _grad_dest(b)
        return dest, not zero_first

    def params(self):
        return [p for p in (self.lin.weight, self.lin.bias) if p is not None]


class QKVUnit:

    def __init__(self, q, k, v):
        self.lins = (q, k, v)
        self._key, self._w, self._wt = None, None, None

    def _ops(self, fresh=False):
        key = tuple((lin.weight.data_ptr(), lin.weight._version, lin.weight.device) for lin in self.lins) + (_engine.PARAM_EPOCH,)
        if (fresh and engine.FORCE_WEIGHT_PREP) or self._key != key:
            w = torch.cat([lin.weight.detach() for lin in self.lins], 0)
            self._w = w.to(_f16)
            self._wt = w.t().contiguous().to(_f16)
            self._key = key
        return self._w, self._wt

    def forward(self, x):
        w, _ = self._ops(fresh=True)
        bias = None
        if self.lins[0].bias is not None:
            bias = torch.cat([lin.bias.detach() for lin in self.lins])
        return tokens.gemm(x, w, bias=bias)

    def backward(self, x, dqkv):
        C = self.lins[0].out_features
        for i, lin in enumerate(self.lins):
            dy = dqkv[..., i * C:(i + 1) * C]
            if lin.weight.requires_grad:
                dw, zero_first = _grad_dest(lin.weight)
                tokens.linear_wgrad(x, dy, dw, zero_first=zero_first)
            if lin.bias is not None and lin.bias.requires_grad:
                db, zero_first = _grad_dest(lin.bias)
                parts = getattr(dqkv, "_sf_bias_parts", None)
                _bias_from_parts(dy, db, not zero_first, None if parts is None else [parts[i]])
        _, wt = self._ops()
        return tokens.gemm(dqkv, wt)

    def params(self):
        return [p for lin in self.lins for p in (lin.weight, lin.bias) if p is not None]


class NormUnit:

    def __init__(self, ln):
        self.ln = ln

    def forward(self, x, side=None):
        return tokens.layernorm_fwd(x, self.ln.weight, self.ln.bias, self.ln.eps, side=side)

    def backward(self, dy, x, mean, rstd, resid=None, sums=None):
        ln = self.ln
        dg, zg = _grad_dest(ln.weight)
        db, zb = _grad_dest(ln.bias)
        assert zg == zb
        return tokens.layernorm_bwd(dy, x, ln.weight, mean, rstd, dg, db, resid=resid, accumulate=not zg, sums=sums)

    def params(self):
        return [self.ln.weight, self.ln.bias]


def _rel_index(q_size, k_size, device):
    q_ratio = max(k_size / q_size, 1.0)
    k_ratio = max(q_size / k_size, 1.0)
    dist = torch.arange(q_size)[:, None] * q_ratio - torch.arange(k_size)[None, :] * k_ratio
    dist += (k_size - 1) * k_ratio
    return dist.long().to(torch.int32).contiguous().to(device)


def _interp_matrix(stored, used, device):
    if stored == used:
        return None
    eye = torch.eye(stored, dtype=torch.float32)
    w = torch.nn.functional.interpolate(eye.reshape(1, stored, stored).permute(0, 2, 1), size=used, mode="linear")
    return w.reshape(stored, used).permute(1, 0).contiguous().to(device)


class AttentionPlan:

    def __init__(self, att, B, thw, device):
        self.B, self.thw = B, tuple(thw)
        self.heads, self.att = att.num_heads, att.dim_out
        self.D = self.att // self.heads
        cls = att.has_cls_embed
        self.cls = int(cls)
        self.dim_in = att.dim_in
        C = self.dim_in if att.pool_first else self.att
        Cw = C // self.heads
        self.gq = self.gk = None
        if att.pool_q is not None:
            kq, sq, pq = tuple(att.pool_q.kernel_size), tuple(att.pool_q.stride), tuple(att.pool_q.padding)
            self.gq = tokens.DwGeom(B, C, Cw, thw, kq, sq, pq, cls)
        if att.pool_k is not None:
            kk, sk, pk = tuple(att.pool_k.kernel_size), tuple(att.pool_k.stride), tuple(att.pool_k.padding)
            self.gk = tokens.DwGeom(B, C, Cw, thw, kk, sk, pk, cls)
        self.q_thw = self.gq.out_thw if self.gq is not None else tuple(thw)
        self.k_thw = self.gk.out_thw if self.gk is not None else tuple(thw)
        self.Nq = self.cls + math.prod(self.q_thw)
        self.Nk = self.cls + math.prod(self.k_thw)
        self.lds = (self.Nk + 31) // 32 * 32
        self.rel = att.rel_pos_spatial and att.rel_pos_temporal
        if att.rel_pos_spatial != att.rel_pos_temporal:
            raise NotImplementedError("spatial and temporal relative positions are used together on this path (MViTv2)")
        (qt, qh, qw), (kt, kh, kw) = self.q_thw, self.k_thw
        rows = (2 * max(qh, kh) - 1, 2 * max(qw, kw) - 1, 2 * max(qt, kt) - 1) if self.rel else (0, 0, 0)
        self.desc = tokens.attn_desc(B, self.heads, self.D, cls, self.q_thw, self.k_thw, *rows)
        self.idx = None
        self.onehot = None
        self.interp = (None, None, None)
        if self.rel:
            self.interp = tuple(_interp_matrix(t.shape[0], r, device)
                                for t, r in zip((att.rel_pos_h, att.rel_pos_w, att.rel_pos_t), rows))
            self.idx = (_rel_index(qh, kh, device), _rel_index(qw, kw, device), _rel_index(qt, kt, device))

# ... 222 lines not shown
    B, Ci = plan.B, plan.dim_in
    Dc = Ci // plan.heads
    dqn, dkn, dvn = _core_backward(att, plan, sv["core"], do)
    dxn = None
    for name, dy, unit, pool, norm, geom, N in (
            ("q", dqn, att._q, att.pool_q, att._norm_q, plan.gq, plan.Nq),
            ("k", dkn, att._k, att.pool_k, att._norm_k, plan.gk, plan.Nk),
            ("v", dvn, att._v, att.pool_v, att._norm_v, plan.gk, plan.Nk)):
        if geom is None:
            dxn = unit.backward(xn, dy, resid=dxn)
            continue
        dxp = unit.backward(sv["x" + name], dy)
        dpool = norm.backward(dxp.view(-1, Dc), sv[name + "p"].view(-1, Dc), *sv["s" + name]).view(B, N, Ci)
        g = tokens.dwconv_dgrad(dpool.view(-1, Ci), pool.weight, geom).view(xn.shape)
        dw, zero_first = _grad_dest(pool.weight)
        tokens.dwconv_wgrad(xn, dpool.view(-1, Ci), geom, dw, zero_first=zero_first)
        dxn = g if dxn is None else dxn.add_(g)
    return dxn


class MultiScaleBlockFn(torch.autograd.Function):

    @staticmethod
    def forward(ctx, x, mod, thw, drop, side, *params):
        engine.record_params(ctx, params)
        att = mod.attn
        B, N, dim = x.shape
        plan = mod._plan(B, thw, x.device)
        xn, m1, r1 = mod._norm1.forward(x, side=side.reader(N) if side is not None else None)
        if att.pool_first:
            qkv = None
            o, sv = attention_forward_pool_first(att, plan, xn)
        else:
            qkv = att._qkv.forward(xn)
            o, sv = attention_forward(att, plan, qkv)
        proj_first = mod._proj is not None and mod.dim_mul_in_att
        proj_last = mod._proj is not None and not mod.dim_mul_in_att
        rside = side
        if proj_first:
            xs = mod._proj.forward(xn)
            rside = None
        else:
            xs = x
        pool = None
        if mod.pool_skip is not None:
            k, s, p = mod.pool_skip.kernel_size, mod.pool_skip.stride, mod.pool_skip.padding
            xres, arg, _ = tokens.token_pool_fwd(xs, B, thw, k, s, p, cls=mod.has_cls_embed)
            pool = (k, s, p, arg, xres)
            if rside is not None:
                rside = ResidSide(cls32=rside.cls_rows())
        else:
            xres = xs
        Nq, Ca = plan.Nq, xres.shape[-1]
        full = bool(getattr(mod, "_resid32_full", False)) and RESID32_FULL
        s1 = side1 = None
        if side is not None:
            s1, side1 = _sum_side(rside if (rside is None or not full or rside.full32 is not None) else None,
                                  B, Nq, Ca, full, x.device)
        if drop is None:
            x1 = att._proj.forward(o, resid=xres, side=s1)
        else:
            x1 = tokens.row_scale_add(att._proj.forward(o), drop[0], xres.shape[1], resid=xres, side=s1)
        xn2, m2, r2 = mod._norm2.forward(x1, side=side1.reader(Nq) if side1 is not None else None)
        h, a = mod.mlp._fc1.forward_gelu(xn2)
        xb = mod._proj.forward(xn2) if proj_last else x1
        s2 = side2 = None
        if side is not None:
            s2, side2 = _sum_side(None if proj_last else side1, B, Nq, xb.shape[-1], full, x.device)
        if drop is None:
            out = mod.mlp._fc2.forward(a, resid=xb, side=s2)
        else:
            out = tokens.row_scale_add(mod.mlp._fc2.forward(a), drop[1], xb.shape[1], resid=xb, side=s2)
        if side is not None:
            side.cls32, side.full32 = side2.cls32, side2.full32
        ctx.drop = drop
        ctx.mod, ctx.plan, ctx.thw = mod, plan, tuple(thw)
        ctx.sv = dict(x=x, xn=xn, s1=(m1, r1), qkv=qkv, att=sv, o=o, pool=pool, x1=x1, xn2=xn2, s2=(m2, r2), h=h, a=a)
        ctx.out_thw = plan.q_thw
        return out

    @staticmethod
    @engine.delivers_grads
    def backward(ctx, dout):
        with tokens.deferred_finalizes():
            dx = MultiScaleBlockFn._backward(ctx, dout)
        _notify(ctx.mod._param_list)
        return (dx, None, None, None, None) + param_grads(ctx, 5)

    @staticmethod
    def _backward(ctx, dout):
        mod, plan, sv = ctx.mod, ctx.plan, ctx.sv
        att = mod.attn
        B = plan.B
        dout = dout.contiguous() if dout.dtype == _f16 else dout.to(_f16).contiguous()
        drop = ctx.drop
        dbr = dout if drop is None else tokens.row_scale_add(dout, drop[1], dout.shape[1])
        proj_first = mod._proj is not None and mod.dim_mul_in_att
        proj_last = mod._proj is not None and not proj_first
        ln_sums = drop is None and not proj_last
        dh, b1_done = mod.mlp._fc2.backward_through_gelu(sv["a"], dbr, sv["h"], consumer_bias=mod.mlp.fc1.bias, bias_done=ln_sums)
        dxn2 = mod.mlp._fc1.backward(sv["xn2"], dh, bias_done=b1_done)
        if proj_last:
            dxn2 = mod._proj.backward(sv["xn2"], dout, resid=dxn2)
            dx1 = mod._norm2.backward(dxn2, sv["x1"], *sv["s2"])
        elif ln_sums:
            dx1 = mod._norm2.backward(dxn2, sv["x1"], *sv["s2"], resid=dout,
                                      sums=(mod.mlp._fc2.bias_sum_dest(), att._proj.bias_sum_dest()))
        else:
            dx1 = mod._norm2.backward(dxn2, sv["x1"], *sv["s2"], resid=dout)
        do = att._proj.backward(sv["o"], dx1 if drop is None else tokens.row_scale_add(dx1, drop[0], dx1.shape[1]),
                                bias_done=ln_sums)
        if att.pool_first:
            dxn = attention_backward_pool_first(att, plan, sv["xn"], sv["att"], do)
        else:
            dqkv = attention_backward(att, plan, sv["qkv"], sv["att"], do)
            dxn = att._qkv.backward(sv["xn"], dqkv)
        dxs = dx1
        if sv["pool"] is not None:
            k, s, p, arg, xres = sv["pool"]
            dxs = tokens.token_pool_bwd(dx1, xres, arg, B, ctx.thw, k, s, p, xres.shape[-1], cls=mod.has_cls_embed)
        if proj_first:
            dxn = mod._proj.backward(sv["xn"], dxs, resid=dxn)
            dx_skip = None
        else:
            dx_skip = dxs
        dx = mod._norm1.backward(dxn, sv["x"], *sv["s1"], resid=dx_skip)
        ctx.sv = None
        return dx


def _attention_sub_forward(sub, plan, x):
    att = sub.attn
    xn, m, r = sub._norm.forward(x)
    if att.pool_first:
        qkv = None
        o, sv = attention_forward_pool_first(att, plan, xn)
    else:
        qkv = att._qkv.forward(xn)
        o, sv = attention_forward(att, plan, qkv)
    return o, dict(x=x, xn=xn, st=(m, r), qkv=qkv, att=sv, o=o)


def _attention_sub_backward(sub, plan, sv, d_out, resid=None):
    att = sub.attn
    do = att._proj.backward(sv["o"], d_out)
    if att.pool_first:
        dxn = attention_backward_pool_first(att, plan, sv["xn"], sv["att"], do)
    else:
        dxn = att._qkv.backward(sv["xn"], attention_backward(att, plan, sv["qkv"], sv["att"], do))
    return sub._norm.backward(dxn, sv["x"], *sv["st"], resid=resid)


def _mlp_sub_forward(sub, x):
    xn, m, r = sub._norm.forward(x)
    h, a = sub.mlp._fc1.forward_gelu(xn)
    return a, dict(x=x, xn=xn, st=(m, r), h=h, a=a)


def _mlp_sub_backward(sub, sv, d_out, resid=None):
    dh, b1_done = sub.mlp._fc2.backward_through_gelu(sv["a"], d_out, sv["h"], consumer_bias=sub.mlp.fc1.bias)
    dxn = sub.mlp._fc1.backward(sv["xn"], dh, bias_done=b1_done)
    return sub._norm.backward(dxn, sv["x"], *sv["st"], resid=resid)


def _f16c(t):
    return t.contiguous() if t.dtype == _f16 else t.to(_f16).contiguous()

# ... 212 lines not shown
```

### slowfast_amd/ops.py

```python
from ctypes import byref, c_int32, c_int64

import torch

from . import lib as _sflib

from .lib import ConvDesc, SfError, get_lib

_f16 = _sflib.act_dtype()


def _triple(v):
    return tuple(v) if isinstance(v, (tuple, list)) else (v, v, v)


def _stream(t):
    if t.is_cuda:
        return torch.cuda.current_stream(t.device).cuda_stream
    if get_lib().backend != "hostsim":
        raise SfError("slowfast_amd kernels need CUDA/HIP tensors (got a CPU tensor and the gfx950 library)")
    return None


def _ptr(t):
    return None if t is None else t.data_ptr()


def cl_empty(shape, device, ld=None, zero=False):
    N, C, T, H, W = shape
    ld = C if ld is None else ld
    base = (torch.zeros if zero else torch.empty)((N, T, H, W, ld), dtype=_f16, device=device)
    return base[..., :C].permute(0, 4, 1, 2, 3)


def cl_ld(x):
    if x.dim() != 5 or x.dtype != _f16:
        raise SfError(f"expected a 5-D fp16 channels-last activation, got {tuple(x.shape)} {x.dtype}")
    N, C, T, H, W = x.shape
    if C > 1 and x.stride(1) != 1:
        raise SfError("activation is not channels-last (channel stride != 1); use ops.to_cl()")
    if W > 1:
        ld = x.stride(4)
    elif H > 1:
        ld = x.stride(3)
    elif T > 1:
        ld = x.stride(2)
    elif N > 1:
        ld = x.stride(0)
    else:
        ld = C
    exp = (T * H * W * ld, 1, H * W * ld, W * ld, ld)
    for dim, size in enumerate(x.shape):
        if size > 1 and x.stride(dim) != exp[dim]:
            raise SfError(f"activation strides {x.stride()} are not channels-last with pitch {ld}")
    if ld < C or ld % 8 or C % 8 or x.data_ptr() % 16:
        raise SfError(f"activation needs C % 8 == 0, pitch % 8 == 0, 16-byte base (C={C}, ld={ld})")
    return ld


def is_cl(x):
    try:
        cl_ld(x)
        return True
    except SfError:
        return False


def rows(x):
    N, C, T, H, W = x.shape
    return N * T * H * W


def ncthw_to_cl(x, Cp=None):
    assert x.dim() == 5 and x.dtype == torch.float32
    x = x.contiguous()
    N, C, T, H, W = x.shape
    Cp = Cp or (C + 7) // 8 * 8
    out = cl_empty((N, Cp, T, H, W), x.device)
    get_lib().call("sf_ncthw_to_cl", x.data_ptr(), N, C, T * H * W, Cp, out.data_ptr(), _stream(x),
                   work=dict(bytes=4.0 * x.numel() + 2.0 * out.numel()))
    return out


def ncthw_to_cl_wpairs(x):
    assert x.dim() == 5 and x.dtype == torch.float32 and x.shape[1] <= 4 and x.shape[4] % 2 == 0
    x = x.contiguous()
    N, C, T, H, W = x.shape
    base = torch.empty((N, T, H, W // 2, 8), dtype=_f16, device=x.device)
    get_lib().call("sf_ncthw_to_cl", x.data_ptr(), N, C, T * H * W, 4, base.data_ptr(), _stream(x),
                   work=dict(bytes=4.0 * x.numel() + 2.0 * base.numel()))
# ... 72 lines not shown
        return None, None, 0
    scale, shift, relu = in_affine
    assert scale.dtype == torch.float32 and shift.dtype == torch.float32
    return scale, shift, int(bool(relu))


def conv_fwd(x, wf, geom, in_affine=None, bias=None, stats=True, out=None):
    assert tuple(x.shape) == geom.in_shape, (x.shape, geom.in_shape)
    ldx = cl_ld(x)
    y = cl_empty(geom.out_shape, x.device) if out is None else out
    ldy = cl_ld(y)
    lib = get_lib()
    d = geom.desc(ldx, ldy)
    part = None
    if stats:
        mt = lib.call("sf_conv_fwd_mtiles", byref(d))
        part = torch.empty((mt, 2, geom.Co), dtype=torch.float32, device=x.device)
    sc, sh, relu = _affine(in_affine)
    lib.call("sf_conv_fwd", byref(d), x.data_ptr(), wf.data_ptr(), _ptr(sc), _ptr(sh), relu, _ptr(bias),
             y.data_ptr(), _ptr(part), _stream(x), work=geom.work(reads_x=1, reads_y=0, writes_y=1))
    return y, part


def conv_fwd_fused(x, wf, geom, bias=None, resid=None, relu=False, out=None):
    assert tuple(x.shape) == geom.in_shape, (x.shape, geom.in_shape)
    y = cl_empty(geom.out_shape, x.device) if out is None else out
    assert tuple(y.shape) == geom.out_shape
    if bias is not None:
        assert bias.dtype == torch.float32 and bias.numel() == geom.Co, "bias must cover the padded channel count"
    ldr = 0
    if resid is not None:
        assert tuple(resid.shape) == geom.out_shape
        ldr = cl_ld(resid)
    get_lib().call("sf_conv_fwd_fused", byref(geom.desc(cl_ld(x), cl_ld(y))), x.data_ptr(), wf.data_ptr(), _ptr(bias),
                   _ptr(resid), ldr, int(bool(relu)), y.data_ptr(), _stream(x),
                   work=geom.work(reads_x=1, reads_y=int(resid is not None), writes_y=1))
    return y


def conv_dgrad(dy, wd, geom, resid=None, out=None, resid_bits=None, bn=None):
    assert tuple(dy.shape) == geom.out_shape
    if resid is not None:
        assert tuple(resid.shape) == geom.in_shape
    if out is not None:
        assert tuple(out.shape) == geom.in_shape
    if bn is not None:
        if not isinstance(bn, dict):
            y0, sc, sh = bn
            bits = None
        else:
            bits, y0 = bn["bits"], bn["y0"]
            sc = sh = None
            assert bits.dtype == torch.uint8 and bits.numel() == rows(y0) * (geom.Ci // 8) and bits.is_contiguous()
        assert tuple(y0.shape) == geom.in_shape
        dx = cl_empty(geom.in_shape, dy.device) if out is None else out
        M = rows(y0)
        cap = (M + 127) // 128
        part = torch.empty((cap, 2, geom.Ci), dtype=torch.float32, device=dy.device)
        nrows = c_int32(0)
        if resid_bits is not None:
            assert resid is not None and resid_bits.dtype == torch.uint8 and resid_bits.numel() == rows(resid) * (geom.Ci // 8)
        get_lib().call("sf_conv_dgrad_bn", byref(geom.desc(cl_ld(dx), cl_ld(dy))), dy.data_ptr(), wd.data_ptr(), _ptr(resid),
                       cl_ld(resid) if resid is not None else 0, _ptr(resid_bits), dx.data_ptr(), _ptr(sc), _ptr(sh), _ptr(bits),
                       y0.data_ptr(), cl_ld(y0), part.data_ptr(), cap, byref(nrows), _stream(dy),
                       work=geom.work(reads_x=1 + int(resid is not None), reads_y=1, writes_x=1))
        return dx, (part[:nrows.value] if nrows.value > 0 else None)
    ldy = cl_ld(dy)
    dx = cl_empty(geom.in_shape, dy.device) if out is None else out
    ldx = cl_ld(dx)
    ldr = cl_ld(resid) if resid is not None else 0
    if resid_bits is not None:
        assert resid is not None and resid_bits.dtype == torch.uint8 and resid_bits.numel() == rows(resid) * (geom.Ci // 8)
    get_lib().call("sf_conv_dgrad", byref(geom.desc(ldx, ldy)), dy.data_ptr(), wd.data_ptr(), _ptr(resid), ldr,
                   _ptr(resid_bits), dx.data_ptr(), _stream(dy),
                   work=geom.work(reads_x=int(resid is not None), reads_y=1, writes_x=1))
    return dx


_workspaces = {}
_retired_workspaces = []


def _workspace(device, nbytes):
    sid = torch.cuda.current_stream(device).cuda_stream if device.type == "cuda" else 0
    k = (device, sid)
    ws = _workspaces.get(k)
    if ws is None or ws.numel() < nbytes:
        if ws is not None:
            _retired_workspaces.append(ws)
        ws = torch.empty(max(int(nbytes * 1.25), 1 << 20), dtype=torch.uint8, device=device)
        _workspaces[k] = ws
    return ws


def conv_wgrad(x, dy, geom, dw, in_affine=None, out_scale=1.0, zero_first=True):
    assert tuple(x.shape) == geom.in_shape and tuple(dy.shape) == geom.out_shape
    assert dw.dtype == torch.float32 and dw.is_contiguous() and dw.numel() == geom.Cow * geom.Cw * geom.taps
    sc, sh, relu = _affine(in_affine)
    lib = get_lib()
    d = geom.desc(cl_ld(x), cl_ld(dy))
    if geom.ws_bytes is None:
        geom.ws_bytes = lib.call("sf_conv_wgrad_workspace", byref(d))
    ws = _workspace(x.device, geom.ws_bytes)
    lib.call("sf_conv_wgrad", byref(d), x.data_ptr(), _ptr(sc), _ptr(sh), relu,
                   dy.data_ptr(), dw.data_ptr(), float(out_scale), int(zero_first), ws.data_ptr(), ws.numel(),
                   _ptr(_wgrad_rowtab(geom, d, x.device)) if sc is None else None, _stream(x),
                   work=geom.work(reads_x=1, reads_y=1))
    return dw


_rowtabs = {}


def _capturing(device):
    return device.type == "cuda" and torch.cuda.is_current_stream_capturing()


def _wgrad_rowtab(geom, d, device):
    nbytes = getattr(geom, "_rowtab_bytes", None)
    if nbytes is None:
        nbytes = geom._rowtab_bytes = get_lib().call("sf_conv_wgrad_rowtab_bytes", byref(d))
    if nbytes <= 0:
        return None
    key = (device, 0, geom.N, geom.Ti, geom.Hi, geom.Wi, geom.To, geom.Ho, geom.Wo, geom.k, geom.s, geom.p, geom.d)
    if key not in _rowtabs:
        tab = torch.empty(nbytes, dtype=torch.uint8, device=device)
        get_lib().call("sf_conv_wgrad_rowtab", byref(d), tab.data_ptr(), _stream(tab))
        if _capturing(device):
            return tab
        if device.type == "cuda":
            torch.cuda.current_stream(device).synchronize()
        _rowtabs[key] = tab
    return _rowtabs[key]


def bn_finalize(part, count, gamma, beta, running_mean, running_var, momentum, eps, training=True, C=None):
    Creal = gamma.numel()
    C = C or (part.shape[2] if part is not None else Creal)
    dev = gamma.device
    scale, shift, mean, rstd = (torch.empty(C, dtype=torch.float32, device=dev) for _ in range(4))
    nblk = part.shape[0] if training else 0
    get_lib().call("sf_bn_finalize", _ptr(part) if training else None, nblk, C, Creal, float(count), gamma.data_ptr(),
                   beta.data_ptr(), _ptr(running_mean), _ptr(running_var), float(momentum), float(eps),
                   scale.data_ptr(), shift.data_ptr(), mean.data_ptr(), rstd.data_ptr(), _stream(gamma))
    return scale, shift, mean, rstd


def bn_act(y, scale=None, shift=None, relu=False, resid=None, rscale=None, rshift=None, out=None, want_mask=False):
    ldy = cl_ld(y)
    N, C, T, H, W = y.shape
    out = cl_empty(y.shape, y.device) if out is None else out
    assert tuple(out.shape) == tuple(y.shape)
    mask = torch.empty((rows(y), C // 8), dtype=torch.uint8, device=y.device) if want_mask else None
    get_lib().call("sf_bn_act", rows(y), C, y.data_ptr(), ldy, _ptr(scale), _ptr(shift), _ptr(resid),
                   cl_ld(resid) if resid is not None else 0, _ptr(rscale), _ptr(rshift), int(bool(relu)),
                   out.data_ptr(), cl_ld(out), _ptr(mask), _stream(y),
                   work=dict(bytes=2.0 * y.numel() * (2 + int(resid is not None) + (1 / 16 if want_mask else 0))))
    return (out, mask) if want_mask else out


def bn_bwd(dz, y, gamma, mean, rstd, dgamma, dbeta, zmask=None, relu_affine=None, inv_loss_scale=1.0,
           accumulate=False, want_g=False, out=None, sync=None, part=None, sample_add=None, coef_only=False):
    lib = get_lib()
    N, C, T, H, W = y.shape
    M = rows(y)
    s = _stream(y)
    fused_part = part
    if fused_part is None:
        nblk = lib.call("sf_bn_bwd_blocks", M, C)
        part = torch.empty((nblk, 2, C), dtype=torch.float32, device=y.device)
    else:
        assert part.dtype == torch.float32 and part.is_contiguous() and tuple(part.shape[1:]) == (2, C)
        nblk = part.shape[0]
    sc, sh = (relu_affine if relu_affine is not None else (None, None))
    relu_self = int(relu_affine is not None)
    bits = zmask is not None and zmask.dtype == torch.uint8
    if bits:
        assert zmask.numel() == M * (C // 8) and zmask.is_contiguous()
    mcost = 0.0 if zmask is None else (1 / 16 if bits else 1.0)
    lddz, ldy, ldm = cl_ld(dz), cl_ld(y), (0 if bits or zmask is None else cl_ld(zmask))
    if fused_part is None:
        lib.call("sf_bn_bwd_reduce", M, C, dz.data_ptr(), lddz, _ptr(zmask), ldm, y.data_ptr(), ldy, _ptr(sc), _ptr(sh),
                 relu_self, part.data_ptr(), s, work=dict(bytes=2.0 * y.numel() * (2 + mcost)))
    coef = torch.empty((3, C), dtype=torch.float32, device=y.device)
    if sync is None:
        lib.call("sf_bn_bwd_finalize", part.data_ptr(), nblk, C, gamma.numel(), float(M), gamma.data_ptr(), mean.data_ptr(),
                 rstd.data_ptr(), float(inv_loss_scale), dgamma.data_ptr(), dbeta.data_ptr(), int(accumulate),
                 coef.data_ptr(), s)
    else:
        import torch.distributed as dist
        group, gsize = sync
        tot = part.sum(0, keepdim=True)
        loc = tot.clone()
        lib.call("sf_bn_bwd_finalize", loc.data_ptr(), 1, C, gamma.numel(), float(M), gamma.data_ptr(), mean.data_ptr(),
                 rstd.data_ptr(), float(inv_loss_scale), dgamma.data_ptr(), dbeta.data_ptr(), int(accumulate),
                 coef.data_ptr(), s)
        dist.all_reduce(tot, group=group)
        scratch = torch.empty((2, gamma.numel()), dtype=torch.float32, device=y.device)
        lib.call("sf_bn_bwd_finalize", tot.data_ptr(), 1, C, gamma.numel(), float(M) * gsize, gamma.data_ptr(),
                 mean.data_ptr(), rstd.data_ptr(), float(inv_loss_scale), scratch[0].data_ptr(), scratch[1].data_ptr(), 0,
                 coef.data_ptr(), s)
    if coef_only:
        return coef
    dy = cl_empty(y.shape, y.device) if out is None else out
    if sample_add is not None:
        assert fused_part is not None and zmask is None and relu_affine is None and not want_g
        assert sample_add.dtype == torch.float32 and sample_add.is_contiguous() and tuple(sample_add.shape) == (N, C)
        lib.call("sf_bn_bwd_apply_sample", M, C, dz.data_ptr(), lddz, y.data_ptr(), ldy, coef.data_ptr(), sample_add.data_ptr(),
                 M // N, dy.data_ptr(), cl_ld(dy), s, work=dict(bytes=2.0 * y.numel() * 3))
        return dy
    g = cl_empty(y.shape, y.device) if want_g else None
    lib.call("sf_bn_bwd_apply", M, C, dz.data_ptr(), lddz, _ptr(zmask), ldm, y.data_ptr(), ldy, _ptr(sc), _ptr(sh),
             relu_self, coef.data_ptr(), dy.data_ptr(), cl_ld(dy), _ptr(g), cl_ld(g) if g is not None else 0, s,
             work=dict(bytes=2.0 * y.numel() * (3 + mcost + int(want_g))))
    return (dy, g) if want_g else dy


def bn_bwd_coef(dz, y, gamma, mean, rstd, dgamma, dbeta, zmask=None, inv_loss_scale=1.0, accumulate=False, part=None):
    return bn_bwd(dz, y, gamma, mean, rstd, dgamma, dbeta, zmask=zmask, inv_loss_scale=inv_loss_scale, accumulate=accumulate,
                  part=part, coef_only=True)


def conv_c_bwd_plan(geom, in_affine=False, mask_bits=True):
    tile_rows, ws = c_int32(0), c_int64(0)
    ok = get_lib().call("sf_conv_c_bwd_plan", byref(geom.desc(geom.Ci, geom.Co)), int(bool(in_affine)), int(bool(mask_bits)),
                        byref(tile_rows), byref(ws))
    return (tile_rows.value, ws.value) if ok == 1 else None


def conv_c_bwd(dz, bits, yc, coef, act, wd, geom, dw, bn=None, out_scale=1.0, zero_first=True, out=None):
    plan = conv_c_bwd_plan(geom)
    assert plan is not None, "conv_c_bwd: the planner rejects this geometry"
    tile_rows, ws_bytes = plan
    assert tuple(act.shape) == geom.in_shape and tuple(dz.shape) == geom.out_shape and tuple(yc.shape) == geom.out_shape
    assert dw.dtype == torch.float32 and dw.is_contiguous() and dw.numel() == geom.Cow * geom.Cw * geom.taps
    M = rows(yc)
    assert bits.dtype == torch.uint8 and bits.is_contiguous() and bits.numel() == M * (geom.Co // 8)
    assert coef.dtype == torch.float32 and coef.is_contiguous() and tuple(coef.shape) == (3, geom.Co)
    d_in = cl_empty(geom.in_shape, dz.device) if out is None else out
    assert tuple(d_in.shape) == geom.in_shape
    part, cap, nrows = None, 0, c_int32(0)
    y0 = sc = sh = None
    if bn is not None:
        y0, sc, sh = bn
        assert tuple(y0.shape) == geom.in_shape
        cap = (M + tile_rows - 1) // tile_rows
        part = torch.empty((cap, 2, geom.Ci), dtype=torch.float32, device=dz.device)
    ws = _workspace(dz.device, ws_bytes)
    W = 2.0 * M * geom.Co
    get_lib().call("sf_conv_c_bwd", byref(geom.desc(cl_ld(act), geom.Co)), dz.data_ptr(), cl_ld(dz), bits.data_ptr(), yc.data_ptr(),
                   cl_ld(yc), coef.data_ptr(), act.data_ptr(), wd.data_ptr(), _ptr(sc), _ptr(sh), _ptr(y0),
                   cl_ld(y0) if y0 is not None else 0, _ptr(part), cap, byref(nrows), d_in.data_ptr(), cl_ld(d_in), dw.data_ptr(),
                   float(out_scale), int(zero_first), ws.data_ptr(), ws.numel(), _stream(dz),
                   work=dict(flops=4.0 * M * geom.Co * geom.Cw,
                             bytes=W * (2 + 1 / 16) + 2.0 * M * geom.Ci * (2 + int(bn is not None))))
    return d_in, (part[:nrows.value] if part is not None and nrows.value > 0 else None)


def _pool_args(y, kernel, stride, padding):
    N, C, T, H, W = y.shape
    (kH, kW), (sH, sW), (pH, pW) = kernel, stride, padding
    return (N, T, H, W, C, kH, kW, sH, sW, pH, pW), ((H + 2 * pH - kH) // sH + 1, (W + 2 * pW - kW) // sW + 1)


def pool_fwd(y, kernel, stride, padding, affine=None, want_argmax=True):
    args, (Ho, Wo) = _pool_args(y, kernel, stride, padding)
    N, C, T, H, W = y.shape
    out = cl_empty((N, C, T, Ho, Wo), y.device)
    arg = torch.empty((N, T, Ho, Wo, C), dtype=torch.uint8, device=y.device) if want_argmax else None
    sc, sh, relu = _affine(affine)
    get_lib().call("sf_pool_fwd", *args, y.data_ptr(), cl_ld(y), _ptr(sc), _ptr(sh), relu, out.data_ptr(),
                   cl_ld(out), _ptr(arg), 0, _stream(y), work=dict(bytes=2.0 * (y.numel() + out.numel())))
    return out, arg


def pool_bwd(in_shape, pooled, argmax, dout, kernel, stride, padding, relu=True):
    N, C, T, H, W = in_shape
    (kH, kW), (sH, sW), (pH, pW) = kernel, stride, padding
    assert tuple(dout.shape) == tuple(pooled.shape)
    g = cl_empty(in_shape, dout.device)
    get_lib().call("sf_pool_bwd", N, T, H, W, C, kH, kW, sH, sW, pH, pW, pooled.data_ptr(), cl_ld(pooled),
                   argmax.data_ptr(), int(bool(relu)), dout.data_ptr(), cl_ld(dout), g.data_ptr(), cl_ld(g), 0,
                   _stream(dout), work=dict(bytes=2.0 * (g.numel() + 2.5 * dout.numel())))
    return g
```

### slowfast_amd/tokens.py

```python
from ctypes import byref, c_int32

import torch

from . import lib as _sflib

from .lib import AttnDesc, ColFinItem, DwDesc, Rows32, SfError, get_lib
from .ops import _ptr, _stream, _workspace

_f16 = _sflib.act_dtype()


def rows_pitch(x):
    if x.dtype != _f16 or x.dim() < 2:
        raise SfError(f"expected an fp16 token tensor, got {tuple(x.shape)} {x.dtype}")
    C = x.shape[-1]
    if C > 1 and x.stride(-1) != 1:
        raise SfError("token tensor must have unit channel stride")
    ld = x.stride(-2) if x.shape[-2] > 1 else max(C, x.stride(-2))
    rows = x.shape[-2]
    for d in range(x.dim() - 3, -1, -1):
        if x.shape[d] > 1 and x.stride(d) != rows * ld:
            raise SfError(f"token tensor rows are not uniformly spaced: shape {tuple(x.shape)} strides {x.stride()}")
        rows *= x.shape[d]
    if ld % 8 or C % 8 or x.data_ptr() % 16:
# ... 3 lines not shown

def _lib_call(name, *args, **kw):
    return get_lib().call(name, *args, **kw)


def _rows32(M, C, period, src=None, dst=None):
    for t in (src, dst):
        if t is not None:
            assert t.dtype == torch.float32 and t.is_contiguous() and t.shape[-1] == C and t.numel() * period == M * C, \
                (tuple(t.shape), M, C, period)
    return Rows32(_ptr(src), _ptr(dst), C, period)


def gemm(a, w16, bias=None, resid=None, out=None, alpha=0.0, side=None):
    M, K, lda = rows_pitch(a)
    N = w16.shape[0]
    assert w16.dtype == _f16 and w16.shape[1] == K and w16.stride(1) == 1
    if out is None:
        out = torch.empty(a.shape[:-1] + (N,), dtype=_f16, device=a.device)
    Mo, No, ldy = rows_pitch(out)
    assert (Mo, No) == (M, N)
    ldr = 0
    if resid is not None:
        Mr, Nr, ldr = rows_pitch(resid)
        assert (Mr, Nr) == (M, N)
    if side is not None:
        assert alpha == 0.0
        d = _rows32(M, N, side[0], side[1], side[2])
        _lib_call("sf_gemm_rows32", M, N, K, a.data_ptr(), lda, w16.data_ptr(), w16.stride(0), _ptr(bias), _ptr(resid), ldr,
                  out.data_ptr(), ldy, byref(d), _stream(a),
                  work=dict(flops=2.0 * M * N * K, bytes=2.0 * (M * K + M * N + N * K)))
        return out
    _lib_call("sf_bgemm", M, N, K, a.data_ptr(), lda, w16.data_ptr(), w16.stride(0), _ptr(bias), _ptr(resid), ldr,
              out.data_ptr(), ldy, 1, 1, 0, 0, 0, 0, 0, 0, 0, 0, 0, float(alpha), _stream(a),
              work=dict(flops=2.0 * M * N * K, bytes=2.0 * (M * K + M * N + N * K)))
    return out


def gemm_gelu(a, w16, bias=None):
    M, K, lda = rows_pitch(a)
    N = w16.shape[0]
    h = torch.empty(a.shape[:-1] + (N,), dtype=_f16, device=a.device)
    act = torch.empty_like(h)
    _lib_call("sf_gemm_act", M, N, K, a.data_ptr(), lda, w16.data_ptr(), w16.stride(0), _ptr(bias), h.data_ptr(), N, 1,
              act.data_ptr(), N, _stream(a), work=dict(flops=2.0 * M * N * K, bytes=2.0 * (M * K + 2 * M * N + N * K)))
    return h, act


def gemm_gelu_grad(dy, wt16, h, dbias=None, accumulate=False):
    M, K, lda = rows_pitch(dy)
    N = wt16.shape[0]
    assert rows_pitch(h)[:2] == (M, N)
    dh = torch.empty(h.shape, dtype=_f16, device=dy.device)
    work = dict(flops=2.0 * M * N * K, bytes=2.0 * (M * K + 2 * M * N + N * K))
    if dbias is None:
        _lib_call("sf_gemm_act", M, N, K, dy.data_ptr(), lda, wt16.data_ptr(), wt16.stride(0), None, dh.data_ptr(), N, 2,
                  h.data_ptr(), rows_pitch(h)[2], _stream(dy), work=work)
        return dh
    cap = (M + 127) // 128
    part = torch.empty((cap, 2, N), dtype=torch.float32, device=dy.device)
    nrows = c_int32(0)
    _lib_call("sf_gemm_act_colsum", M, N, K, dy.data_ptr(), lda, wt16.data_ptr(), wt16.stride(0), None, dh.data_ptr(), N, 2,
              h.data_ptr(), rows_pitch(h)[2], part.data_ptr(), cap, byref(nrows), _stream(dy), work=work)
    colsum_finalize(part[:nrows.value], N, N, dbias, None, 1.0, accumulate)
    return dh


def bgemm_heads(a, a_strides, M, K, lda, w, w_strides, N, ldw, out, o_strides, ldy, B, heads, resid=None,
                r_strides=(0, 0), ldr=0, resid_row0=0, alpha=0.0):
    _lib_call("sf_bgemm", M, N, K, a.data_ptr(), lda, w.data_ptr(), ldw, None, _ptr(resid), ldr, out.data_ptr(), ldy,
              B * heads, heads, a_strides[0], a_strides[1], w_strides[0], w_strides[1], o_strides[0], o_strides[1],
              r_strides[0], r_strides[1], resid_row0, float(alpha), _stream(a),
              work=dict(flops=2.0 * B * heads * M * N * K, bytes=2.0 * B * heads * (M * K + N * K + M * N)))
    return out


def bgemm_tn_heads(p, p_strides, ldp, x, x_strides, ldx, M, R, Kc, out, o_strides, ldo, B, heads, scale=1.0):
    _lib_call("sf_bgemm_tn", M, R, Kc, p.data_ptr(), ldp, x.data_ptr(), ldx, out.data_ptr(), ldo, float(scale),
              B * heads, heads, p_strides[0], p_strides[1], x_strides[0], x_strides[1], o_strides[0], o_strides[1],
              _stream(p), work=dict(flops=2.0 * B * heads * M * R * Kc, bytes=2.0 * B * heads * (M * R + M * Kc + R * Kc)))
    return out


def linear_wgrad(x, dy, dw, zero_first=True):
    from . import ops
    M, K, ldx = rows_pitch(x)
    Md, N, ldy = rows_pitch(dy)
    assert Md == M and tuple(dw.shape) == (N, K) and dw.dtype == torch.float32 and dw.is_contiguous()
    geom = _linear_geom(M, K, N)
    lib = get_lib()
    d = geom.desc(ldx, ldy)
    if geom.ws_bytes is None:
        geom.ws_bytes = lib.call("sf_conv_wgrad_workspace", byref(d))
    ws = _workspace(x.device, geom.ws_bytes)
    lib.call("sf_conv_wgrad", byref(d), x.data_ptr(), None, None, 0, dy.data_ptr(), dw.data_ptr(), 1.0, int(zero_first),
             ws.data_ptr(), ws.numel(), _ptr(ops._wgrad_rowtab(geom, d, x.device)), _stream(x),
             work=dict(flops=2.0 * M * N * K, bytes=2.0 * M * (N + K)))
    return dw


_geoms = {}


def _linear_geom(M, K, N):
    from . import ops
    key = (M, K, N)
    g = _geoms.get(key)
    if g is None:
        g = _geoms[key] = ops.ConvGeom((1, K, 1, 1, M), N, (1, 1, 1))
    return g


def layernorm_fwd(x, gamma, beta, eps, out=None, save_stats=True, side=None):
    M, C, ldx = rows_pitch(x)
    y = torch.empty(x.shape, dtype=_f16, device=x.device) if out is None else out
    _, _, ldy = rows_pitch(y)
    mean = torch.empty(M, dtype=torch.float32, device=x.device) if save_stats else None
    rstd = torch.empty(M, dtype=torch.float32, device=x.device) if save_stats else None
    if side is not None:
        d = _rows32(M, C, side[0], side[1], None)
        _lib_call("sf_layernorm_fwd_rows32", M, C, x.data_ptr(), ldx, gamma.data_ptr(), beta.data_ptr(), float(eps),
                  y.data_ptr(), ldy, _ptr(mean), _ptr(rstd), byref(d), _stream(x), work=dict(bytes=4.0 * M * C))
        return y, mean, rstd
    _lib_call("sf_layernorm_fwd", M, C, x.data_ptr(), ldx, gamma.data_ptr(), beta.data_ptr(), float(eps), y.data_ptr(),
              ldy, _ptr(mean), _ptr(rstd), _stream(x), work=dict(bytes=4.0 * M * C))
    return y, mean, rstd


_pending_fin = None
_FIN_MAX_ROWS = 2048


class deferred_finalizes:

    def __enter__(self):
        global _pending_fin
        self._outer = _pending_fin
        if _pending_fin is None:
            _pending_fin = []
        return self

    def __exit__(self, *exc):
        global _pending_fin
        if self._outer is None and _pending_fin is not None:
            try:
                if exc[0] is None:
                    flush_finalizes()
            finally:
                _pending_fin = None
        return False


def flush_finalizes():
    global _pending_fin
    items = _pending_fin
    if not items:
        return
    _pending_fin = []
    _finalize_batch(items)


def _finalize_batch(items):
    arr = (ColFinItem * len(items))()
    part0 = items[0][0]
    cur = torch.cuda.current_stream(part0.device) if part0.is_cuda else None
    for i, (part, C, fold, out0, out1, scale, accumulate, stride, st) in enumerate(items):
        arr[i] = ColFinItem(part.data_ptr(), part.shape[0], C, fold, _ptr(out0), _ptr(out1), float(scale), int(accumulate),
                            int(stride))
        if st is not None and cur is not None and st != cur:
            cur.wait_stream(st)
    _lib_call("sf_colsum_finalize_batch", arr, len(items), _stream(part0))


def colsum_finalize(part, C, fold, out0, out1, scale=1.0, accumulate=False, row_stride=1):
    if _pending_fin is not None and part.shape[0] <= _FIN_MAX_ROWS:
        outs = [o.data_ptr() for o in (out0, out1) if o is not None]
        for it in _pending_fin:
            if any(o is not None and o.data_ptr() in outs for o in (it[3], it[4])):
                flush_finalizes()
                break
# ... 509 lines not shown
```

### slowfast_amd/x3d.py

```python
import math
import os
from ctypes import byref

import torch
import torch.nn as nn

from . import lib as _sflib

from . import engine, ops, tokens
from .engine import BNState, ConvUnit, StemConvUnit, _grad_dest, _notify, _sync_of, as_cl, bn_statistics, param_grads
from .lib import get_lib
from .registry import MODEL_REGISTRY
from .resblocks import ResStage, _TRANS
from .video_models import get_norm, init_weights

_f16 = _sflib.act_dtype()

SE_FROM_STATS = os.environ.get("SF_SE_FROM_STATS", "1") != "0"
GATE_ONE_PASS = os.environ.get("SF_GATE_ONE_PASS", "1") != "0"


def _pad8(c):
    return (c + 7) // 8 * 8

# ... 153 lines not shown

    @staticmethod
    def forward(ctx, x, mod, *params):
        engine.record_params(ctx, params)
        xy, dw, bn = mod._xy, mod._dw, mod._bn
        xcl = xy.prepare_input(x)
        y1, _ = xy.forward(xcl, None, mod.training)
        y2, part, g = dw.forward(y1, stats=True)
        st = bn.finalize(part, g.rows_out, y2.shape[1], mod.training)
        out = ops.bn_act(y2, st.scale, st.shift, relu=True)
        if engine.CAPTURE is not None:
            engine.CAPTURE.append({"kind": "x3d_stem", "mod": mod, "raw": [y2], "bn": [(st.scale, st.shift)]})
        ctx.mod, ctx.sv = mod, (xcl, y1, y2, st)
        return out

    @staticmethod
    @engine.delivers_grads
    def backward(ctx, dout):
        mod = ctx.mod
        xcl, y1, y2, st = ctx.sv
        dy2 = mod._bn.backward(as_cl(dout), y2, st, relu_self=True)
        dy1 = mod._dw.backward(y1, dy2, need_dx=True)
        mod._xy.backward(xcl, None, dy1, need_dx=False)
        _notify(list(mod.parameters()))
        ctx.sv = None
        return (None, None) + param_grads(ctx, 2)


class X3DBlockFn(torch.autograd.Function):

    @staticmethod
    def forward(ctx, x, mod, *params):
        engine.record_params(ctx, params)
        ctx.prev_bn = getattr(x, "_sf_block_bn", None) if engine.BN_FUSE_REDUCE else None
        x = as_cl(x)
        t = mod.branch2
        tr = mod.training
        A, C, P = t._a, t._c, mod._proj
        ya, sa = A.forward(x, None, tr)
        za = ops.bn_act(ya, sa.scale, sa.shift, relu=True)
        yb, part, g = t._b.forward(za, stats=True)
        nrow = getattr(g, "stat_sample_rows", 0) if (t._se is not None and SE_FROM_STATS) else 0
        ysum = part.view(yb.shape[0], nrow, 2, -1)[:, :, 0].sum(1) if nrow > 0 else None
        sb = t._b_bn.finalize(part, g.rows_out, yb.shape[1], tr)
        gate = se = None
        if t._se is not None:
            if ysum is not None:
                m = torch.addcmul(sb.shift, ysum, sb.scale, value=float(yb.shape[0]) / float(g.rows_out))
            else:
                m = sample_mean(yb, sb.scale, sb.shift, relu=False)
            h, gate = t._se.gate_fwd(m)
            se = (m, h)
        zb = gate_act_fwd(yb, sb.scale, sb.shift, gate, t._swish_inner)
        yc, sc = C.forward(zb, None, tr)
        if P is not None:
            y1, s1 = P.forward(x, None, tr)
            out, bits = ops.bn_act(yc, sc.scale, sc.shift, relu=True, resid=y1, rscale=s1.scale, rshift=s1.shift,
                                   want_mask=True)
        else:
            y1, s1 = None, None
            out, bits = ops.bn_act(yc, sc.scale, sc.shift, relu=True, resid=x, want_mask=True)
        if engine.CAPTURE is not None:
            engine.CAPTURE.append({"kind": "x3d_block", "mod": mod, "raw": [ya], "bn": [(sa.scale, sa.shift)], "out": out,
                                   "se_h": None if se is None else se[1]})
        ctx.mod = mod
        ctx.sv = dict(ya=ya, sa=sa, za=za, yb=yb, sb=sb, gate=gate, se=se, zb=zb, yc=yc, sc=sc, y1=y1, s1=s1, bits=bits,
                      ysum=ysum)
        ctx.save_for_backward(x)
        if engine.BN_FUSE_REDUCE and tr:
            out._sf_block_bn = {"bits": bits, "y0": yc, "sync": _sync_of(C.bn) is not None}
        return out

    @staticmethod
    @engine.delivers_grads
    def backward(ctx, dout):
        mod, sv = ctx.mod, ctx.sv
        t = mod.branch2
        A, C, P = t._a, t._c, mod._proj
        (x,) = ctx.saved_tensors
        part_c = engine.tagged_bn_part(dout, sv["yc"])
        dout = as_cl(dout)
        need_dx = ctx.needs_input_grad[0]
        bits = sv["bits"]
        dyc = C.bn_backward(dout, sv["yc"], sv["sc"], zmask=bits, part=part_c)
        if P is not None:
            dy1 = P.bn_backward(dout, sv["y1"], sv["s1"], zmask=bits)
        dzb = C.backward(sv["zb"], None, dyc, need_dx=True)
        dyb = gate_bn_backward(t, sv["yb"], sv["sb"], sv["gate"], sv["se"], sv["ysum"], dzb)
        dza = t._b.backward(sv["za"], dyb, need_dx=True)
        dya = A.bn_backward(dza, sv["ya"], sv["sa"], relu_self=True)
        prev = ctx.prev_bn if need_dx else None
        if prev is not None and prev["sync"]:
            prev = None
        if P is not None:
            dx1 = P.backward(x, None, dy1, need_dx=need_dx)
            dx = A.backward(x, None, dya, need_dx=need_dx, resid=dx1, bn_fuse=prev)
        else:
            dx = A.backward(x, None, dya, need_dx=need_dx, resid=dout, resid_bits=bits, bn_fuse=prev)
        if prev is not None:
            dx, pc = dx
            if pc is not None:
                engine.tag_bn_part(dx, prev["y0"], pc)
        _notify(mod._param_list)
        ctx.sv = ctx.prev_bn = None
        return (dx, None) + param_grads(ctx, 2)


class X3DHeadPoolFn(torch.autograd.Function):

    @staticmethod
    def forward(ctx, x, mod, *params):
        engine.record_params(ctx, params)
        x = as_cl(x)
        unit = mod._conv5
        y, st = unit.forward(x, None, mod.training)
        m = sample_mean(y, st.scale, st.shift, relu=True)
        if engine.CAPTURE is not None:
            engine.CAPTURE.append({"kind": "x3d_head", "mod": mod, "raw": [y], "bn": [(st.scale, st.shift)]})
        ctx.mod, ctx.y, ctx.st = mod, y, st
        ctx.save_for_backward(x)
        return m[:, :unit.conv.out_channels].contiguous()

    @staticmethod
    @engine.delivers_grads
    def backward(ctx, dm):
        mod, y, st = ctx.mod, ctx.y, ctx.st
        unit = mod._conv5
        (x,) = ctx.saved_tensors
        N, Cp = y.shape[:2]
        S = ops.rows(y) // N
        dmp = torch.zeros((N, Cp), dtype=torch.float32, device=dm.device)
        dmp[:, :dm.shape[1]] = dm / S
        dz2d = dmp.to(_f16)[:, None, :].expand(N, S, Cp).contiguous().view(N * S, Cp)
        dz = cl5d(dz2d, N, Cp, y.shape[2:])
        dy = unit.bn_backward(dz, y, st, relu_self=True)
        dx = unit.backward(x, None, dy, need_dx=ctx.needs_input_grad[0])
        _notify(unit.params())
        ctx.y = None
        return (dx, None) + param_grads(ctx, 2)


class X3DStem(nn.Module):
    def __init__(self, dim_in, dim_out, kernel, stride, padding, inplace_relu=True, eps=1e-5, bn_mmt=0.1,
                 norm_module=nn.BatchNorm3d):
        super().__init__()
        self.kernel, self.stride, self.padding = kernel, stride, padding
        self.inplace_relu, self.eps, self.bn_mmt = inplace_relu, eps, bn_mmt
        self.conv_xy = nn.Conv3d(dim_in, dim_out, kernel_size=(1, kernel[1], kernel[2]), stride=(1, stride[1], stride[2]),
                                 padding=(0, padding[1], padding[2]), bias=False)
        self.conv = nn.Conv3d(dim_out, dim_out, kernel_size=(kernel[0], 1, 1), stride=(stride[0], 1, 1),
                              padding=(padding[0], 0, 0), bias=False, groups=dim_out)
        self.bn = norm_module(num_features=dim_out, eps=eps, momentum=bn_mmt)
        self.relu = nn.ReLU(inplace_relu)
        self._xy, self._dw, self._bn = StemConvUnit(self.conv_xy, None), DwUnit(self.conv), BNUnit(self.bn)

    def forward(self, x):
        return X3DStemFn.apply(x, self, *self.parameters())


class SE(nn.Module):

    @staticmethod
    def _round_width(width, multiplier, min_width=8, divisor=8):
        if not multiplier:
            return width
        width *= multiplier
        min_width = min_width or divisor
        width_out = max(min_width, int(width + divisor / 2) // divisor * divisor)
        if width_out < 0.9 * width:
            width_out += divisor
        return int(width_out)

    def __init__(self, dim_in, ratio, relu_act=True):
        super().__init__()
        if not relu_act:
            raise NotImplementedError("SE with a Swish squeeze activation is not used by any X3D config")
        self.avg_pool = nn.AdaptiveAvgPool3d((1, 1, 1))
        dim_fc = self._round_width(dim_in, ratio)
        self.fc1 = nn.Conv3d(dim_in, dim_fc, 1, bias=True)
        self.fc1_act = nn.ReLU()
        self.fc2 = nn.Conv3d(dim_fc, dim_in, 1, bias=True)
        self.fc2_sig = nn.Sigmoid()
        self.dim_in, self.dim_fc = dim_in, dim_fc

    def gate_fwd(self, m):
# ... 221 lines not shown
```

Baseline: 903.4 clips/s.

## Defer per-conv wgrad split reductions and batch them into one launch per block

Splits the wgrad and fused c-bwd entry points into a partials phase that returns a reduce descriptor instead of launching the split-K reduction. A scope around each residual block's backward collects these descriptors and flushes them through a single batched reduce kernel, with up to 8 items per launch. The goal is fewer small kernel launches and reduce kernels with better occupancy. In exchange, the per-call workspace must stay live until the flush, which risks aliasing if the shared workspace is reused before the batched reduce runs. Since fwd+bwd runs under a HIP graph, launch overhead matters less, so any gain would come mainly from fuller reduce grids.

Measured after the change: 905.1 clips/s (median of 3 runs). Within noise of the previous version (+0.2%).

```diff
diff --git a/include/sfamd.h b/include/sfamd.h
--- a/include/sfamd.h
+++ b/include/sfamd.h
@@ -6,7 +6,7 @@
 extern "C" {
 #endif
 
-#define SF_ABI_VERSION 34
+#define SF_ABI_VERSION 35
 typedef void* sf_stream_t;
 
 typedef struct sf_conv_desc {
@@ -65,6 +65,24 @@
                   const void* bn_y, int32_t bn_ldy, float* bn_part, int32_t bn_part_rows, int32_t* bn_rows, void* d_in,
                   int32_t ld_in, float* dw, float out_scale, int zero_first, void* workspace, int64_t workspace_bytes,
                   sf_stream_t stream);
+typedef struct sf_wgrad_reduce_item {
+    const float* ws;
+    float* dw;
+    int32_t slabs, Co_pad, Kpad, slice4;
+    int32_t Co, Ci, Cw, taps, Ktot;
+    float out_scale;
+    int32_t zero_first;
+    int32_t pad;
+} sf_wgrad_reduce_item;
+int sf_conv_wgrad_partials(const sf_conv_desc* d, const void* x, const float* in_scale, const float* in_shift, int in_relu,
+                           const void* dy, float* dw, float out_scale, int zero_first, void* workspace,
+                           int64_t workspace_bytes, const void* rowtab, sf_wgrad_reduce_item* item, sf_stream_t stream);
+int sf_conv_c_bwd_partials(const sf_conv_desc* d, const void* dz, int32_t lddz, const void* mask_bits, const void* yc,
+                           int32_t ldyc, const float* coef, const void* act, const void* wd, const float* bn_scale,
+                           const float* bn_shift, const void* bn_y, int32_t bn_ldy, float* bn_part, int32_t bn_part_rows,
+                           int32_t* bn_rows, void* d_in, int32_t ld_in, float* dw, float out_scale, int zero_first,
+                           void* workspace, int64_t workspace_bytes, sf_wgrad_reduce_item* item, sf_stream_t stream);
+int sf_wgrad_reduce_batch(const sf_wgrad_reduce_item* items, int32_t n, sf_stream_t stream);
 
 int sf_bn_finalize(float* part, int32_t nblk, int32_t C, int32_t Creal, float count, const float* gamma, const float* beta,
                    float* running_mean, float* running_var, float momentum, float eps, float* scale, float* shift,
diff --git a/slowfast_amd/csrc/sf_api.hip b/slowfast_amd/csrc/sf_api.hip
--- a/slowfast_amd/csrc/sf_api.hip
+++ b/slowfast_amd/csrc/sf_api.hip
@@ -647,18 +647,29 @@
         default: hipLaunchKernelGGL((sf_wgrad_kernel<16, 16, 32, 4>), grid, block, 0, s, p); break;
     }
 }
-static void launch_wgrad_reduce(const sf_conv_desc* d, const float* ws, int slabs, int Co_pad, int Kpad, bool slice4, float* dw,
-                                float out_scale, int zero_first, hipStream_t s) {
-    WgradReduceParams r;
+static void fill_wgrad_reduce_item(sf_wgrad_reduce_item* it, const sf_conv_desc* d, const float* ws, int slabs, int Co_pad, int Kpad,
+                                   bool slice4, float* dw, float out_scale, int zero_first) {
+    memset(it, 0, sizeof(*it));
+    it->ws = ws; it->dw = dw; it->slabs = slabs; it->Co_pad = Co_pad; it->Kpad = Kpad; it->slice4 = slice4 ? 1 : 0;
+    it->Co = d->Cow ? d->Cow : d->Co; it->Ci = d->Ci; it->Cw = d->Cw; it->taps = d->kT * d->kH * d->kW;
+    it->Ktot = slice4 ? d->kT * d->kH * 32 : it->taps * d->Ci;
+    it->out_scale = out_scale; it->zero_first = zero_first ? 1 : 0;
+}
+static int wgrad_reduce_params(const sf_wgrad_reduce_item& it, WgradReduceParams& r) {
     memset(&r, 0, sizeof(r));
-    r.ws = ws; r.splits = slabs; r.Co = d->Cow ? d->Cow : d->Co; r.Co_pad = Co_pad; r.Kpad = Kpad;
-    r.taps = d->kT * d->kH * d->kW; r.Ktot = r.taps * d->Ci; r.fdC = make_fastdiv(d->Ci); r.dw = dw; r.Cw = d->Cw;
-    if (slice4) { r.slice4 = 1; r.Ktot = d->kT * d->kH * 32; }
-    r.out_scale = out_scale; r.accumulate = zero_first ? 0 : 1;
+    r.ws = it.ws; r.splits = it.slabs; r.Co = it.Co; r.Co_pad = it.Co_pad; r.Kpad = it.Kpad;
+    r.taps = it.taps; r.Ktot = it.Ktot; r.fdC = make_fastdiv(it.Ci); r.dw = it.dw; r.Cw = it.Cw;
+    r.slice4 = it.slice4;
+    r.out_scale = it.out_scale; r.accumulate = it.zero_first ? 0 : 1;
     const int64_t total = (int64_t)r.Co * r.Kpad / 4;
     r.lanes = 1;
     while (r.lanes < 32 && r.lanes * 4 <= r.splits) r.lanes *= 2;
-    hipLaunchKernelGGL(sf_wgrad_reduce_kernel, dim3(cdiv(total, SF_THREADS / r.lanes)), dim3(SF_THREADS), 0, s, r);
+    return (int)cdiv(total, SF_THREADS / r.lanes);
+}
+static void launch_wgrad_reduce(const sf_wgrad_reduce_item& it, hipStream_t s) {
+    WgradReduceParams r;
+    const int blocks = wgrad_reduce_params(it, r);
+    hipLaunchKernelGGL(sf_wgrad_reduce_kernel, dim3(blocks), dim3(SF_THREADS), 0, s, r);
 }
 
 enum WgradPath { WGRAD_GEN1, WGRAD_ROWTAB, WGRAD_STEM };
@@ -812,9 +823,10 @@
     return plain > affine ? plain : affine;
 }
 
-extern "C" int sf_conv_wgrad(const sf_conv_desc* d, const void* x, const float* in_scale, const float* in_shift,
-                             int in_relu, const void* dy, float* dw, float out_scale, int zero_first,
-                             void* workspace, int64_t workspace_bytes, const void* rowtab, sf_stream_t stream) {
+static int conv_wgrad_partials_impl(const sf_conv_desc* d, const void* x, const float* in_scale, const float* in_shift,
+                                    int in_relu, const void* dy, float* dw, float out_scale, int zero_first,
+                                    void* workspace, int64_t workspace_bytes, const void* rowtab, sf_wgrad_reduce_item* item,
+                                    sf_stream_t stream) {
     if (check_desc(d)) return -1;
     REQUIRE(x && dy && dw && workspace, "sf_conv_wgrad: null pointer");
     REQUIRE((in_scale == nullptr) == (in_shift == nullptr), "sf_conv_wgrad: in_scale/in_shift must come together");
@@ -881,8 +893,48 @@
         launch_wgrad1(w.BMW, p, dim3(w.tiles_k, w.tiles_c, w.splits), s);
     }
     if (check_launch("wgrad")) return -1;
-    launch_wgrad_reduce(d, slabs, w.slabs, w.Co_pad, w.Kpad, w.path == WGRAD_STEM && w.stem.thin3, dw, out_scale, zero_first, s);
+    fill_wgrad_reduce_item(item, d, slabs, w.slabs, w.Co_pad, w.Kpad, w.path == WGRAD_STEM && w.stem.thin3, dw, out_scale, zero_first);
+    return 0;
+}
+
+extern "C" int sf_conv_wgrad(const sf_conv_desc* d, const void* x, const float* in_scale, const float* in_shift,
+                             int in_relu, const void* dy, float* dw, float out_scale, int zero_first,
+                             void* workspace, int64_t workspace_bytes, const void* rowtab, sf_stream_t stream) {
+    sf_wgrad_reduce_item it;
+    if (conv_wgrad_partials_impl(d, x, in_scale, in_shift, in_relu, dy, dw, out_scale, zero_first, workspace, workspace_bytes,
+                                 rowtab, &it, stream)) return -1;
+    launch_wgrad_reduce(it, (hipStream_t)stream);
     return check_launch("wgrad_reduce");
+}
+
+extern "C" int sf_conv_wgrad_partials(const sf_conv_desc* d, const void* x, const float* in_scale, const float* in_shift,
+                                      int in_relu, const void* dy, float* dw, float out_scale, int zero_first,
+                                      void* workspace, int64_t workspace_bytes, const void* rowtab,
+                                      sf_wgrad_reduce_item* item, sf_stream_t stream) {
+    REQUIRE(item, "sf_conv_wgrad_partials: null item");
+    return conv_wgrad_partials_impl(d, x, in_scale, in_shift, in_relu, dy, dw, out_scale, zero_first, workspace, workspace_bytes,
+                                    rowtab, item, stream);
+}
+
+extern "C" int sf_wgrad_reduce_batch(const sf_wgrad_reduce_item* items, int32_t n, sf_stream_t stream) {
+    REQUIRE(items && n > 0, "sf_wgrad_reduce_batch: no items");
+    for (int i = 0; i < n; ++i) {
+        const sf_wgrad_reduce_item& it = items[i];
+        REQUIRE(it.ws && it.dw && ((uintptr_t)it.ws & 15) == 0, "sf_wgrad_reduce_batch: item %d: null or misaligned pointer", i);
+        REQUIRE(it.slabs > 0 && it.Co > 0 && it.Co <= it.Co_pad && it.Kpad > 0 && it.Kpad % 4 == 0 && it.Ci > 0 && it.Cw > 0 &&
+                it.Cw <= it.Ci && it.taps > 0 && it.Ktot > 0 && it.Ktot <= it.Kpad, "sf_wgrad_reduce_batch: bad item %d", i);
+        REQUIRE(it.slice4 ? it.Ktot % 32 == 0 && it.Ktot / 32 * 3 == it.taps : it.Ktot == it.taps * it.Ci,
+                "sf_wgrad_reduce_batch: item %d: Ktot does not match taps x Ci", i);
+        for (int j = 0; j < i; ++j) REQUIRE(items[j].dw != it.dw, "sf_wgrad_reduce_batch: items %d and %d share dw", j, i);
+    }
+    for (int i0 = 0; i0 < n; i0 += SF_WGRAD_RED_BATCH) {
+        WgradReduceBatch b;
+        memset(&b, 0, sizeof(b));
+        b.n = n - i0 < SF_WGRAD_RED_BATCH ? n - i0 : SF_WGRAD_RED_BATCH;
+        for (int i = 0; i < b.n; ++i) b.first[i + 1] = b.first[i] + wgrad_reduce_params(items[i0 + i], b.item[i]);
+        hipLaunchKernelGGL(sf_wgrad_reduce_batch_kernel, dim3(b.first[b.n]), dim3(SF_THREADS), 0, (hipStream_t)stream, b);
+    }
+    return check_launch("wgrad_reduce_batch");
 }
 
 struct CbwdPlan {
@@ -936,11 +988,11 @@
     return w.ok ? 1 : 0;
 }
 
-extern "C" int sf_conv_c_bwd(const sf_conv_desc* d, const void* dz, int32_t lddz, const void* mask_bits, const void* yc,
-                             int32_t ldyc, const float* coef, const void* act, const void* wd, const float* bn_scale,
-                             const float* bn_shift, const void* bn_y, int32_t bn_ldy, float* bn_part, int32_t bn_part_rows,
-                             int32_t* bn_rows, void* d_in, int32_t ld_in, float* dw, float out_scale, int zero_first,
-                             void* workspace, int64_t workspace_bytes, sf_stream_t stream) {
+static int conv_c_bwd_partials_impl(const sf_conv_desc* d, const void* dz, int32_t lddz, const void* mask_bits, const void* yc,
+                                    int32_t ldyc, const float* coef, const void* act, const void* wd, const float* bn_scale,
+                                    const float* bn_shift, const void* bn_y, int32_t bn_ldy, float* bn_part, int32_t bn_part_rows,
+                                    int32_t* bn_rows, void* d_in, int32_t ld_in, float* dw, float out_scale, int zero_first,
+                                    void* workspace, int64_t workspace_bytes, sf_wgrad_reduce_item* item, sf_stream_t stream) {
     if (check_desc(d)) return -1;
     REQUIRE(dz && mask_bits && yc && coef && act && wd && d_in && dw && workspace, "sf_conv_c_bwd: null pointer");
     const CbwdPlan w = plan_cbwd(d, false, true);
@@ -986,8 +1038,33 @@
     SF_CBWD_FOR_SHAPE(w.cip, w.cop, hipLaunchKernelGGL((sf_cbwd_kernel<CIP_, COP_>), dim3(wgs), dim3(SF_THREADS), 0, s, p));
     if (check_launch("conv_c_bwd")) return -1;
     if (bn_rows) *bn_rows = fuse ? ntiles : 0;
-    launch_wgrad_reduce(d, (const float*)workspace, wgs, w.cop, w.cip, false, dw, out_scale, zero_first, s);
+    fill_wgrad_reduce_item(item, d, (const float*)workspace, wgs, w.cop, w.cip, false, dw, out_scale, zero_first);
+    return 0;
+}
+
+extern "C" int sf_conv_c_bwd(const sf_conv_desc* d, const void* dz, int32_t lddz, const void* mask_bits, const void* yc,
+                             int32_t ldyc, const float* coef, const void* act, const void* wd, const float* bn_scale,
+                             const float* bn_shift, const void* bn_y, int32_t bn_ldy, float* bn_part, int32_t bn_part_rows,
+                             int32_t* bn_rows, void* d_in, int32_t ld_in, float* dw, float out_scale, int zero_first,
+                             void* workspace, int64_t workspace_bytes, sf_stream_t stream) {
+    sf_wgrad_reduce_item it;
+    if (conv_c_bwd_partials_impl(d, dz, lddz, mask_bits, yc, ldyc, coef, act, wd, bn_scale, bn_shift, bn_y, bn_ldy, bn_part,
+                                 bn_part_rows, bn_rows, d_in, ld_in, dw, out_scale, zero_first, workspace, workspace_bytes, &it,
+                                 stream)) return -1;
+    launch_wgrad_reduce(it, (hipStream_t)stream);
     return check_launch("conv_c_bwd_reduce");
+}
+
+extern "C" int sf_conv_c_bwd_partials(const sf_conv_desc* d, const void* dz, int32_t lddz, const void* mask_bits, const void* yc,
+                                      int32_t ldyc, const float* coef, const void* act, const void* wd, const float* bn_scale,
+                                      const float* bn_shift, const void* bn_y, int32_t bn_ldy, float* bn_part,
+                                      int32_t bn_part_rows, int32_t* bn_rows, void* d_in, int32_t ld_in, float* dw,
+                                      float out_scale, int zero_first, void* workspace, int64_t workspace_bytes,
+                                      sf_wgrad_reduce_item* item, sf_stream_t stream) {
+    REQUIRE(item, "sf_conv_c_bwd_partials: null item");
+    return conv_c_bwd_partials_impl(d, dz, lddz, mask_bits, yc, ldyc, coef, act, wd, bn_scale, bn_shift, bn_y, bn_ldy, bn_part,
+                                    bn_part_rows, bn_rows, d_in, ld_in, dw, out_scale, zero_first, workspace, workspace_bytes, item,
+                                    stream);
 }
 
 static RowTile make_rowtile(int64_t M, int C, int max_blocks, dim3& grid) {
diff --git a/slowfast_amd/csrc/sf_igemm.h b/slowfast_amd/csrc/sf_igemm.h
--- a/slowfast_amd/csrc/sf_igemm.h
+++ b/slowfast_amd/csrc/sf_igemm.h
@@ -426,13 +426,12 @@
     int slice4;
 };
 
-__global__ __launch_bounds__(SF_THREADS) void sf_wgrad_reduce_kernel(WgradReduceParams p) {
-    __shared__ f32x4 s_acc[SF_THREADS];
+__device__ __forceinline__ void wgrad_reduce_block(const WgradReduceParams& p, int blk, f32x4* s_acc) {
     const int L = p.lanes, E = SF_THREADS / L;
     const int e = threadIdx.x % E, z0 = threadIdx.x / E;
     const int64_t total = (int64_t)p.Co * p.Kpad;
     const int64_t slab = (int64_t)p.Co_pad * p.Kpad;
-    const int64_t idx = ((int64_t)blockIdx.x * E + e) * 4;
+    const int64_t idx = ((int64_t)blk * E + e) * 4;
     f32x4 a0 = {0.f, 0.f, 0.f, 0.f}, a1 = a0, a2 = a0, a3 = a0;
     if (idx < total) {
         const float* src = p.ws + idx;
@@ -474,6 +473,23 @@
         }
     }
 }
+__global__ __launch_bounds__(SF_THREADS) void sf_wgrad_reduce_kernel(WgradReduceParams p) {
+    __shared__ f32x4 s_acc[SF_THREADS];
+    wgrad_reduce_block(p, (int)blockIdx.x, s_acc);
+}
+
+#define SF_WGRAD_RED_BATCH 8
+struct WgradReduceBatch {
+    WgradReduceParams item[SF_WGRAD_RED_BATCH];
+    int first[SF_WGRAD_RED_BATCH + 1];
+    int n;
+};
+__global__ __launch_bounds__(SF_THREADS) void sf_wgrad_reduce_batch_kernel(WgradReduceBatch b) {
+    __shared__ f32x4 s_acc[SF_THREADS];
+    int i = 0;
+    while (i + 1 < b.n && (int)blockIdx.x >= b.first[i + 1]) ++i;
+    wgrad_reduce_block(b.item[i], (int)blockIdx.x - b.first[i], s_acc);
+}
 
 template <class V>
 __device__ __forceinline__ f16x4 as_f16x4(V v) {
diff --git a/slowfast_amd/engine.py b/slowfast_amd/engine.py
--- a/slowfast_amd/engine.py
+++ b/slowfast_amd/engine.py
@@ -653,36 +653,37 @@
         raw, y1, act, bits = ctx.raw
         bn, s1 = ctx.bn
         last = len(units) - 1
-        part_c = tagged_bn_part(dout, raw[last])
-        dout = as_cl(dout)
-        need_dx = ctx.needs_input_grad[0]
-        cgeom = units[last].fused_c_geom(act[last - 1]) if last > 0 else None
-        if cgeom is None:
-            dy = units[last].bn_backward(dout, raw[last], bn[last], zmask=bits, part=part_c)
-        if P is not None:
-            dy1 = P.bn_backward(dout, y1, s1, zmask=bits)
-        for i in range(last, 0, -1):
-            part = None
-            if i == last and cgeom is not None:
-                inner = (raw[i - 1], bn[i - 1]) if BN_FUSE_REDUCE and _sync_of(units[i - 1].bn) is None else None
-                d_in, part = units[i].fused_c_backward(cgeom, act[i - 1], dout, raw[i], bn[i], bits, part=part_c, bn_fuse=inner)
-            elif BN_FUSE_REDUCE and _sync_of(units[i - 1].bn) is None:
-                d_in, part = units[i].backward(act[i - 1], None, dy, need_dx=True, bn_fuse=(raw[i - 1], bn[i - 1]))
+        with ops.wgrad_reduce_scope(dout.device):
+            part_c = tagged_bn_part(dout, raw[last])
+            dout = as_cl(dout)
+            need_dx = ctx.needs_input_grad[0]
+            cgeom = units[last].fused_c_geom(act[last - 1]) if last > 0 else None
+            if cgeom is None:
+                dy = units[last].bn_backward(dout, raw[last], bn[last], zmask=bits, part=part_c)
+            if P is not None:
+                dy1 = P.bn_backward(dout, y1, s1, zmask=bits)
+            for i in range(last, 0, -1):
+                part = None
+                if i == last and cgeom is not None:
+                    inner = (raw[i - 1], bn[i - 1]) if BN_FUSE_REDUCE and _sync_of(units[i - 1].bn) is None else None
+                    d_in, part = units[i].fused_c_backward(cgeom, act[i - 1], dout, raw[i], bn[i], bits, part=part_c, bn_fuse=inner)
+                elif BN_FUSE_REDUCE and _sync_of(units[i - 1].bn) is None:
+                    d_in, part = units[i].backward(act[i - 1], None, dy, need_dx=True, bn_fuse=(raw[i - 1], bn[i - 1]))
+                else:
+                    d_in = units[i].backward(act[i - 1], None, dy, need_dx=True)
+                dy = units[i - 1].bn_backward(d_in, raw[i - 1], bn[i - 1], relu_self=True, part=part)
+            prev = ctx.prev_bn if need_dx else None
+            if prev is not None and prev["sync"]:
+                prev = None
+            if P is not None:
+                dx1 = P.backward(x, None, dy1, need_dx=need_dx)
+                dx = units[0].backward(x, None, dy, need_dx=need_dx, resid=dx1, bn_fuse=prev)
             else:
-                d_in = units[i].backward(act[i - 1], None, dy, need_dx=True)
-            dy = units[i - 1].bn_backward(d_in, raw[i - 1], bn[i - 1], relu_self=True, part=part)
-        prev = ctx.prev_bn if need_dx else None
-        if prev is not None and prev["sync"]:
-            prev = None
-        if P is not None:
-            dx1 = P.backward(x, None, dy1, need_dx=need_dx)
-            dx = units[0].backward(x, None, dy, need_dx=need_dx, resid=dx1, bn_fuse=prev)
-        else:
-            dx = units[0].backward(x, None, dy, need_dx=need_dx, resid=dout, resid_bits=bits, bn_fuse=prev)
-        if prev is not None:
-            dx, pc = dx
-            if pc is not None:
-                tag_bn_part(dx, prev["y0"], pc)
+                dx = units[0].backward(x, None, dy, need_dx=need_dx, resid=dout, resid_bits=bits, bn_fuse=prev)
+            if prev is not None:
+                dx, pc = dx
+                if pc is not None:
+                    tag_bn_part(dx, prev["y0"], pc)
         _notify(mod._param_list)
         ctx.raw = ctx.bn = ctx.prev_bn = None
         return (dx, None) + param_grads(ctx, 2)
diff --git a/slowfast_amd/lib.py b/slowfast_amd/lib.py
--- a/slowfast_amd/lib.py
+++ b/slowfast_amd/lib.py
@@ -3,7 +3,7 @@
 from ctypes import POINTER, Structure, c_char_p, c_float, c_int, c_int32, c_int64, c_void_p
 
 _HERE = os.path.dirname(os.path.abspath(__file__))
-ABI_VERSION = 34
+ABI_VERSION = 35
 ACT_MODE = os.environ.get("SF_ACT_DTYPE", "fp16").lower()
 if ACT_MODE not in ("fp16", "bf16"):
     raise ValueError(f"SF_ACT_DTYPE={ACT_MODE!r}: expected fp16 or bf16")
@@ -48,6 +48,13 @@
 
     _fields_ = [("part", c_void_p), ("nblk", c_int32), ("C", c_int32), ("fold", c_int32), ("out0", c_void_p),
                 ("out1", c_void_p), ("scale", c_float), ("accumulate", c_int32), ("row_stride", c_int32)]
+
+
+class WgradReduceItem(Structure):
+
+    _fields_ = [("ws", c_void_p), ("dw", c_void_p)] + [(n, c_int32) for n in (
+        "slabs", "Co_pad", "Kpad", "slice4", "Co", "Ci", "Cw", "taps", "Ktot")] + [
+        ("out_scale", c_float), ("zero_first", c_int32), ("pad", c_int32)]
 
 
 class AttnDesc(Structure):
@@ -79,6 +86,11 @@
     "sf_conv_wgrad_rowtab_bytes": (c_int64, [POINTER(ConvDesc)]),
     "sf_conv_wgrad_rowtab": (c_int, [POINTER(ConvDesc), _P, _P]),
     "sf_conv_wgrad": (c_int, [POINTER(ConvDesc), _P, _F, _F, c_int, _P, _F, c_float, c_int, _P, c_int64, _P, _P]),
+    "sf_conv_wgrad_partials": (c_int, [POINTER(ConvDesc), _P, _F, _F, c_int, _P, _F, c_float, c_int, _P, c_int64, _P,
+                                       POINTER(WgradReduceItem), _P]),
+    "sf_conv_c_bwd_partials": (c_int, [POINTER(ConvDesc), _P, c_int32, _P, _P, c_int32, _F, _P, _P, _F, _F, _P, c_int32, _F, c_int32,
+                                       POINTER(c_int32), _P, c_int32, _F, c_float, c_int, _P, c_int64, POINTER(WgradReduceItem), _P]),
+    "sf_wgrad_reduce_batch": (c_int, [POINTER(WgradReduceItem), c_int32, _P]),
     "sf_conv_c_bwd_plan": (c_int, [POINTER(ConvDesc), c_int, c_int, POINTER(c_int32), POINTER(c_int64)]),
     "sf_conv_c_bwd": (c_int, [POINTER(ConvDesc), _P, c_int32, _P, _P, c_int32, _F, _P, _P, _F, _F, _P, c_int32, _F, c_int32,
                               POINTER(c_int32), _P, c_int32, _F, c_float, c_int, _P, c_int64, _P]),
diff --git a/slowfast_amd/mvit_engine.py b/slowfast_amd/mvit_engine.py
--- a/slowfast_amd/mvit_engine.py
+++ b/slowfast_amd/mvit_engine.py
@@ -5,7 +5,7 @@
 
 from . import lib as _sflib
 
-from . import engine, tokens
+from . import engine, ops, tokens
 from . import engine as _engine
 from .engine import _grad_dest, _notify, param_grads
 
@@ -97,7 +97,7 @@
         lin = self.lin
         if lin.weight.requires_grad:
             dw, zero_first = _grad_dest(lin.weight)
-            tokens.linear_wgrad(x, dy, dw, zero_first=zero_first)
+            tokens.linear_wgrad(x, dy, dw, zero_first=zero_first, defer=True)
         if lin.bias is not None and lin.bias.requires_grad and not bias_done:
             db, zero_first = _grad_dest(lin.bias)
             tokens.bias_grad(dy, db, accumulate=not zero_first)
@@ -111,7 +111,7 @@
         lin = self.lin
         if lin.weight.requires_grad:
             dw, zero_first = _grad_dest(lin.weight)
-            tokens.linear_wgrad(x, dy, dw, zero_first=zero_first)
+            tokens.linear_wgrad(x, dy, dw, zero_first=zero_first, defer=True)
         if lin.bias is not None and lin.bias.requires_grad and not bias_done:
             db, zero_first = _grad_dest(lin.bias)
             _bias_from_parts(dy, db, not zero_first, getattr(dy, "_sf_bias_parts", None))
@@ -159,7 +159,7 @@
             dy = dqkv[..., i * C:(i + 1) * C]
             if lin.weight.requires_grad:
                 dw, zero_first = _grad_dest(lin.weight)
-                tokens.linear_wgrad(x, dy, dw, zero_first=zero_first)
+                tokens.linear_wgrad(x, dy, dw, zero_first=zero_first, defer=True)
             if lin.bias is not None and lin.bias.requires_grad:
                 db, zero_first = _grad_dest(lin.bias)
                 parts = getattr(dqkv, "_sf_bias_parts", None)
@@ -548,7 +548,7 @@
     @staticmethod
     @engine.delivers_grads
     def backward(ctx, dout):
-        with tokens.deferred_finalizes():
+        with tokens.deferred_finalizes(), ops.wgrad_reduce_scope(dout.device):
             dx = MultiScaleBlockFn._backward(ctx, dout)
         _notify(ctx.mod._param_list)
         return (dx, None, None, None, None) + param_grads(ctx, 5)
diff --git a/slowfast_amd/ops.py b/slowfast_amd/ops.py
--- a/slowfast_amd/ops.py
+++ b/slowfast_amd/ops.py
@@ -1,10 +1,11 @@
+import os
 from ctypes import byref, c_int32, c_int64
 
 import torch
 
 from . import lib as _sflib
 
-from .lib import ConvDesc, SfError, get_lib
+from .lib import ConvDesc, SfError, WgradReduceItem, get_lib
 
 _f16 = _sflib.act_dtype()
 
@@ -243,15 +244,71 @@
 
 
 def _workspace(device, nbytes):
-    sid = torch.cuda.current_stream(device).cuda_stream if device.type == "cuda" else 0
-    k = (device, sid)
+    k = _ws_key(device)
+    st, off = _wgrad_pending.get(k), 0
+    if st is not None:
+        if not st.items:
+            st.cursor = 0
+        elif st.cursor + nbytes > WGRAD_PENDING_CAP:
+            _flush_wgrad_reduces(st)
+        off = st.cursor
+        st.cursor = off + (int(nbytes) + 255) // 256 * 256
     ws = _workspaces.get(k)
-    if ws is None or ws.numel() < nbytes:
+    if ws is None or ws.numel() < off + nbytes:
         if ws is not None:
             _retired_workspaces.append(ws)
-        ws = torch.empty(max(int(nbytes * 1.25), 1 << 20), dtype=torch.uint8, device=device)
+        ws = torch.empty(max(int((off + nbytes) * 1.25), 1 << 20), dtype=torch.uint8, device=device)
         _workspaces[k] = ws
-    return ws
+    return ws if st is None else ws[off:off + int(nbytes)]
+
+
+def _ws_key(device):
+    return (device, torch.cuda.current_stream(device).cuda_stream if device.type == "cuda" else 0)
+
+
+BLOCK_BATCH = os.environ.get("SF_BLOCK_BATCH", "1") != "0"
+WGRAD_PENDING_CAP = 512 << 20
+_wgrad_pending = {}
+
+
+class _PendingReduces:
+    def __init__(self):
+        self.items, self.cursor = [], 0
+
+
+class wgrad_reduce_scope:
+    def __init__(self, device):
+        self.key = _ws_key(device)
+
+    def __enter__(self):
+        self._outer = self.key in _wgrad_pending
+        if not self._outer and BLOCK_BATCH:
+            _wgrad_pending[self.key] = _PendingReduces()
+        return self
+
+    def __exit__(self, *exc):
+        if not self._outer:
+            st = _wgrad_pending.pop(self.key, None)
+            if st is not None and exc[0] is None:
+                _flush_wgrad_reduces(st, self.key[1])
+        return False
+
+
+def _flush_wgrad_reduces(st, stream=None):
+    items, st.items, st.cursor = st.items, [], 0
+    if not items:
+        return
+    arr = (WgradReduceItem * len(items))(*[it for it, _ in items])
+    if stream is None:
+        stream = _stream(items[0][1])
+    get_lib().call("sf_wgrad_reduce_batch", arr, len(items), stream or None)
+
+
+def _pending_for(dw):
+    st = _wgrad_pending.get(_ws_key(dw.device)) if _wgrad_pending else None
+    if st is not None and any(d.data_ptr() == dw.data_ptr() for _, d in st.items):
+        _flush_wgrad_reduces(st)
+    return st
 
 
 def conv_wgrad(x, dy, geom, dw, in_affine=None, out_scale=1.0, zero_first=True):
@@ -262,11 +319,19 @@
     d = geom.desc(cl_ld(x), cl_ld(dy))
     if geom.ws_bytes is None:
         geom.ws_bytes = lib.call("sf_conv_wgrad_workspace", byref(d))
+    st = _pending_for(dw)
     ws = _workspace(x.device, geom.ws_bytes)
-    lib.call("sf_conv_wgrad", byref(d), x.data_ptr(), _ptr(sc), _ptr(sh), relu,
-                   dy.data_ptr(), dw.data_ptr(), float(out_scale), int(zero_first), ws.data_ptr(), ws.numel(),
-                   _ptr(_wgrad_rowtab(geom, d, x.device)) if sc is None else None, _stream(x),
-                   work=geom.work(reads_x=1, reads_y=1))
+    rowtab = _ptr(_wgrad_rowtab(geom, d, x.device)) if sc is None else None
+    if st is None:
+        lib.call("sf_conv_wgrad", byref(d), x.data_ptr(), _ptr(sc), _ptr(sh), relu,
+                 dy.data_ptr(), dw.data_ptr(), float(out_scale), int(zero_first), ws.data_ptr(), ws.numel(),
+                 rowtab, _stream(x), work=geom.work(reads_x=1, reads_y=1))
+        return dw
+    item = WgradReduceItem()
+    lib.call("sf_conv_wgrad_partials", byref(d), x.data_ptr(), _ptr(sc), _ptr(sh), relu,
+             dy.data_ptr(), dw.data_ptr(), float(out_scale), int(zero_first), ws.data_ptr(), ws.numel(),
+             rowtab, byref(item), _stream(x), work=geom.work(reads_x=1, reads_y=1))
+    st.items.append((item, dw))
     return dw
 
 
@@ -407,14 +472,20 @@
         assert tuple(y0.shape) == geom.in_shape
         cap = (M + tile_rows - 1) // tile_rows
         part = torch.empty((cap, 2, geom.Ci), dtype=torch.float32, device=dz.device)
+    st = _pending_for(dw)
     ws = _workspace(dz.device, ws_bytes)
     W = 2.0 * M * geom.Co
-    get_lib().call("sf_conv_c_bwd", byref(geom.desc(cl_ld(act), geom.Co)), dz.data_ptr(), cl_ld(dz), bits.data_ptr(), yc.data_ptr(),
-                   cl_ld(yc), coef.data_ptr(), act.data_ptr(), wd.data_ptr(), _ptr(sc), _ptr(sh), _ptr(y0),
-                   cl_ld(y0) if y0 is not None else 0, _ptr(part), cap, byref(nrows), d_in.data_ptr(), cl_ld(d_in), dw.data_ptr(),
-                   float(out_scale), int(zero_first), ws.data_ptr(), ws.numel(), _stream(dz),
-                   work=dict(flops=4.0 * M * geom.Co * geom.Cw,
-                             bytes=W * (2 + 1 / 16) + 2.0 * M * geom.Ci * (2 + int(bn is not None))))
+    item = WgradReduceItem() if st is not None else None
+    args = (byref(geom.desc(cl_ld(act), geom.Co)), dz.data_ptr(), cl_ld(dz), bits.data_ptr(), yc.data_ptr(),
+            cl_ld(yc), coef.data_ptr(), act.data_ptr(), wd.data_ptr(), _ptr(sc), _ptr(sh), _ptr(y0),
+            cl_ld(y0) if y0 is not None else 0, _ptr(part), cap, byref(nrows), d_in.data_ptr(), cl_ld(d_in), dw.data_ptr(),
+            float(out_scale), int(zero_first), ws.data_ptr(), ws.numel())
+    work = dict(flops=4.0 * M * geom.Co * geom.Cw, bytes=W * (2 + 1 / 16) + 2.0 * M * geom.Ci * (2 + int(bn is not None)))
+    if st is None:
+        get_lib().call("sf_conv_c_bwd", *args, _stream(dz), work=work)
+    else:
+        get_lib().call("sf_conv_c_bwd_partials", *args, byref(item), _stream(dz), work=work)
+        st.items.append((item, dw))
     return d_in, (part[:nrows.value] if part is not None and nrows.value > 0 else None)
 
 
diff --git a/slowfast_amd/tokens.py b/slowfast_amd/tokens.py
--- a/slowfast_amd/tokens.py
+++ b/slowfast_amd/tokens.py
@@ -109,7 +109,7 @@
     return out
 
 
-def linear_wgrad(x, dy, dw, zero_first=True):
+def linear_wgrad(x, dy, dw, zero_first=True, defer=False):
     from . import ops
     M, K, ldx = rows_pitch(x)
     Md, N, ldy = rows_pitch(dy)
@@ -119,10 +119,16 @@
     d = geom.desc(ldx, ldy)
     if geom.ws_bytes is None:
         geom.ws_bytes = lib.call("sf_conv_wgrad_workspace", byref(d))
+    st = ops._pending_for(dw)
+    if not defer:
+        st = None
     ws = _workspace(x.device, geom.ws_bytes)
-    lib.call("sf_conv_wgrad", byref(d), x.data_ptr(), None, None, 0, dy.data_ptr(), dw.data_ptr(), 1.0, int(zero_first),
-             ws.data_ptr(), ws.numel(), _ptr(ops._wgrad_rowtab(geom, d, x.device)), _stream(x),
-             work=dict(flops=2.0 * M * N * K, bytes=2.0 * M * (N + K)))
+    item = ops.WgradReduceItem() if st is not None else None
+    lib.call("sf_conv_wgrad" if st is None else "sf_conv_wgrad_partials", byref(d), x.data_ptr(), None, None, 0, dy.data_ptr(),
+             dw.data_ptr(), 1.0, int(zero_first), ws.data_ptr(), ws.numel(), _ptr(ops._wgrad_rowtab(geom, d, x.device)),
+             *(() if st is None else (byref(item),)), _stream(x), work=dict(flops=2.0 * M * N * K, bytes=2.0 * M * (N + K)))
+    if st is not None:
+        st.items.append((item, dw))
     return dw
 
 
diff --git a/slowfast_amd/x3d.py b/slowfast_amd/x3d.py
--- a/slowfast_amd/x3d.py
+++ b/slowfast_amd/x3d.py
@@ -259,25 +259,26 @@
         dout = as_cl(dout)
         need_dx = ctx.needs_input_grad[0]
         bits = sv["bits"]
-        dyc = C.bn_backward(dout, sv["yc"], sv["sc"], zmask=bits, part=part_c)
-        if P is not None:
-            dy1 = P.bn_backward(dout, sv["y1"], sv["s1"], zmask=bits)
-        dzb = C.backward(sv["zb"], None, dyc, need_dx=True)
-        dyb = gate_bn_backward(t, sv["yb"], sv["sb"], sv["gate"], sv["se"], sv["ysum"], dzb)
-        dza = t._b.backward(sv["za"], dyb, need_dx=True)
-        dya = A.bn_backward(dza, sv["ya"], sv["sa"], relu_self=True)
-        prev = ctx.prev_bn if need_dx else None
-        if prev is not None and prev["sync"]:
-            prev = None
-        if P is not None:
-            dx1 = P.backward(x, None, dy1, need_dx=need_dx)
-            dx = A.backward(x, None, dya, need_dx=need_dx, resid=dx1, bn_fuse=prev)
-        else:
-            dx = A.backward(x, None, dya, need_dx=need_dx, resid=dout, resid_bits=bits, bn_fuse=prev)
-        if prev is not None:
-            dx, pc = dx
-            if pc is not None:
-                engine.tag_bn_part(dx, prev["y0"], pc)
+        with ops.wgrad_reduce_scope(dout.device):
+            dyc = C.bn_backward(dout, sv["yc"], sv["sc"], zmask=bits, part=part_c)
+            if P is not None:
+                dy1 = P.bn_backward(dout, sv["y1"], sv["s1"], zmask=bits)
+            dzb = C.backward(sv["zb"], None, dyc, need_dx=True)
+            dyb = gate_bn_backward(t, sv["yb"], sv["sb"], sv["gate"], sv["se"], sv["ysum"], dzb)
+            dza = t._b.backward(sv["za"], dyb, need_dx=True)
+            dya = A.bn_backward(dza, sv["ya"], sv["sa"], relu_self=True)
+            prev = ctx.prev_bn if need_dx else None
+            if prev is not None and prev["sync"]:
+                prev = None
+            if P is not None:
+                dx1 = P.backward(x, None, dy1, need_dx=need_dx)
+                dx = A.backward(x, None, dya, need_dx=need_dx, resid=dx1, bn_fuse=prev)
+            else:
+                dx = A.backward(x, None, dya, need_dx=need_dx, resid=dout, resid_bits=bits, bn_fuse=prev)
+            if prev is not None:
+                dx, pc = dx
+                if pc is not None:
+                    engine.tag_bn_part(dx, prev["y0"], pc)
         _notify(mod._param_list)
         ctx.sv = ctx.prev_bn = None
         return (dx, None) + param_grads(ctx, 2)
```
